# nv-nguyen/nope

Hardware: NVIDIA H100
Metric: pose-hypotheses/sec @256x256 (UNet sweep + l2 score + top-5) (higher is better)
Workload: dtype fp16

## Files before the change

### nope_b200/csrc/conv_tc.cuh

```cuda
#pragma once
#include "common.cuh"
#include <cudaTypedefs.h>

namespace nope {

constexpr int kBM = 128;
constexpr int kBK = 64;
constexpr int kMaxSeg = 64;
constexpr int kMaxAMaps = 8;
constexpr int kConvThreads = 384;
constexpr int kEpiWarps = 8;

struct ConvSeg {
  int16_t map;
  int16_t dy, dx;
  int16_t nchunks;
  int32_t wcol1;
};

struct GnFuse {
  const float* gamma;
  const float* beta;
  int G;
  int cpg;
  int gpt;
  int tpg;
  int mt;
  int ipt;
  int expected;
  int hw_shift;
  float inv_cnt;
  float eps;
  int silu;
  const __half* pb;
  int pb_stride, pb_off;
  int has_res;
  int res_div, res_base;
  int n_img;
  uint2* xpart;
  unsigned epoch;
  float2* emit;
  int emit_parts;
  __half* out_lo;
  const __half* res_lo;
  const float2* pre_stats;
  int pre_parts;
  float pre_inv_cnt;
  const float* pre_w1;
  const float* pre_wb;
  int dbg;
  unsigned long long* ts;
};

struct ConvParams {
  CUtensorMap amap[kMaxAMaps];
  int n_amaps;
  CUtensorMap bmap;
  CUtensorMap bmap2;
  CUtensorMap omap[4];
  CUtensorMap rmap;
  GnFuse gn;
  const float* bias;
  int bf16;
  int l2_prefetch;
  int n_par;
  int n_tiles_par;
  int src_w, src_hw;
  int relu;
  const __half* res_hi;
  const __half* res_lo;
  __half* out_lo;
  float* out_f32;
  int geglu;
  float2* stats;
  int stats_hw;
  int stats_noct;
  int n_total;
  int m_valid;
  int nseg;
  int ksteps;
  int m_tiles, n_tiles;
  int tiles_per_img;
  int h_cnt, b_cnt;
  ConvSeg seg[kMaxSeg];
};

template <int BN, int STAGES>
struct ConvSmem {
  static constexpr int kABytes = kBM * kBK * 2;
  static constexpr int kBBytes = BN * kBK * 2;
  static constexpr int kStageBytes = kABytes + kBBytes;
  static constexpr int kOutBytes = (BN / 64) * kBM * 128;
  static constexpr int kBarOffset = STAGES * kStageBytes + kOutBytes;
  static constexpr int kBiasOffset = kBarOffset + 256;
  static constexpr int kTotal = kBiasOffset + BN * 4 + 1024;
  static_assert(STAGES * kStageBytes >= kBM * (BN + 4) * 4, "the fp32 accumulator tile must fit in the operand ring");
  static_assert(kTotal <= 227 * 1024, "shared memory per block");
};

__device__ __forceinline__ void conv_tile_coords(const ConvParams& p, int m_tile, int& b0,
                                                 int& y0) {
  if (p.tiles_per_img > 0) {
    b0 = m_tile / p.tiles_per_img;
    y0 = (m_tile - b0 * p.tiles_per_img) * p.h_cnt;
  } else {
    b0 = m_tile * p.b_cnt;
    y0 = 0;
  }
}

__host__ __device__ constexpr int acc_ld(int BN) { return BN + 4; }

template <int NS, int STAGES, int kStageBytes, int kABytes, bool BF>
__device__ __forceinline__ void conv_mma_loop(const ConvParams& p, const uint8_t* smem, uint64_t* full_bar,
                                              uint64_t* empty_bar, int& stage, uint32_t& phase, int wg,
                                              float (&d0)[NS / 2], float (&d1)[NS / 2]) {
  const int lane = threadIdx.x & 31;
  int prev = -1;
  for (int ks = 0; ks < p.ksteps; ++ks) {
    mbar_wait(&full_bar[stage], phase);
    const uint8_t* sa = smem + stage * kStageBytes;
    const uint64_t adesc = wg_desc_k(sa);
    const uint64_t bdesc = wg_desc_k(sa + kABytes + wg * NS * 128);
    wgmma_fence();
#pragma unroll
    for (int k = 0; k < kBK / 16; ++k) {
      const uint32_t acc = (ks | k) != 0 ? 1u : 0u;
      Wgmma<NS, BF>::mma(d0, adesc + 2 * k, bdesc + 2 * k, acc);
      Wgmma<NS, BF>::mma(d1, adesc + 512 + 2 * k, bdesc + 2 * k, acc);
    }
    wgmma_commit();
    wgmma_wait<1>();
    if (prev >= 0 && lane == 0) mbar_arrive(&empty_bar[prev]);
    prev = stage;
    if (++stage == STAGES) { stage = 0; phase ^= 1; }
  }
  wgmma_wait<0>();
  if (prev >= 0 && lane == 0) mbar_arrive(&empty_bar[prev]);
}

template <int BN, int NW, int STAGES, int kStageBytes, int kABytes>
__device__ __forceinline__ void conv_mma_tile(const ConvParams& p, uint8_t* smem, uint64_t* full_bar,
                                              uint64_t* empty_bar, int& stage, uint32_t& phase, float* s_acc) {
  constexpr int NS = BN / NW;
  static_assert(NS % 32 == 0 && NS <= 128, "columns per warpgroup");
  const int wg = (threadIdx.x >> 7) - 1;
  float d0[NS / 2], d1[NS / 2];
#pragma unroll
  for (int i = 0; i < NS / 2; ++i) { d0[i] = 0.f; d1[i] = 0.f; }
  if (p.bf16) conv_mma_loop<NS, STAGES, kStageBytes, kABytes, true>(p, smem, full_bar, empty_bar, stage, phase, wg, d0, d1);
  else conv_mma_loop<NS, STAGES, kStageBytes, kABytes, false>(p, smem, full_bar, empty_bar, stage, phase, wg, d0, d1);
  asm volatile("bar.sync 2, %0;" ::"n"(NW * 128) : "memory");
  wg_store_acc<NS>(s_acc, acc_ld(BN), wg * NS, d0, d1);
  asm volatile("bar.sync 2, %0;" ::"n"(NW * 128) : "memory");
}

__device__ __forceinline__ void acc_release(uint64_t* tempty, int lane) {
  fence_proxy_async_smem();
  __syncwarp();
  if (lane == 0) mbar_arrive(tempty);
}

template <int kSeg>
__device__ __forceinline__ int butterfly8(float (&v)[8], int lane) {
  static_assert(kSeg == 16 || kSeg == 32, "segment must be 16 or 32 lanes");
  constexpr int m0 = kSeg / 2, m1 = kSeg / 4, m2 = kSeg / 8;
  {
    const bool up = (lane & m0) != 0;
#pragma unroll
    for (int i = 0; i < 4; ++i) {
      const float send = up ? v[i] : v[i + 4];
      const float keep = up ? v[i + 4] : v[i];
      v[i] = keep + __shfl_xor_sync(0xffffffffu, send, m0);
    }
  }
  {
    const bool up = (lane & m1) != 0;
#pragma unroll
    for (int i = 0; i < 2; ++i) {
      const float send = up ? v[i] : v[i + 2];
      const float keep = up ? v[i + 2] : v[i];
      v[i] = keep + __shfl_xor_sync(0xffffffffu, send, m1);
    }
  }
  {
    const bool up = (lane & m2) != 0;
    const float send = up ? v[0] : v[1];
    const float keep = up ? v[1] : v[0];
    v[0] = keep + __shfl_xor_sync(0xffffffffu, send, m2);
  }
#pragma unroll
  for (int m = m2 / 2; m > 0; m >>= 1) v[0] += __shfl_xor_sync(0xffffffffu, v[0], m);
  return ((lane & m0) ? 4 : 0) + ((lane & m1) ? 2 : 0) + ((lane & m2) ? 1 : 0);
}

template <int BN>
struct ResPrefetch {
  uint4 v[BN / 64][4];
  int next_m_tile, next_n_chan0;
  __device__ __forceinline__ void load_sub(const ConvParams& p, int cc, int m_tile, int n_chan0, int e, int lane) {
    const int q = e & 3, hh = e >> 2;
    const int grow = m_tile * kBM + q * 32 + lane;
    if (p.res_hi && m_tile >= 0 && grow < p.m_valid) {
      const size_t roff = (size_t)grow * p.n_total + n_chan0 + cc * 64 + hh * 32;
#pragma unroll
      for (int j = 0; j < 4; ++j) v[cc][j] = *reinterpret_cast<const uint4*>(p.res_hi + roff + j * 8);
    }
  }
  __device__ __forceinline__ void load(const ConvParams& p, int m_tile, int n_chan0, int e, int lane) {
#pragma unroll
    for (int cc = 0; cc < BN / 64; ++cc) load_sub(p, cc, m_tile, n_chan0, e, lane);
  }
};

template <int BN, bool EXTRAS>
__device__ __forceinline__ void conv_epilogue_tile(const ConvParams& p, uint8_t* out_stage,
                                                   const float* s_bias, const float* s_acc, int m_tile,
                                                   int n_chan0, int e, int lane,
                                                   ResPrefetch<BN>* pre = nullptr, int par = 0) {
  const int q = e & 3, hh = e >> 2;
  const int row = q * 32 + lane;
  const float* a_row = s_acc + row * acc_ld(BN) + hh * 32;
  const int grow = m_tile * kBM + row;
  const bool row_ok = grow < p.m_valid;
  size_t opix = (size_t)grow;
  if (EXTRAS && p.n_par == 4) {
    const int img = grow / p.src_hw, r = grow - img * p.src_hw;
    const int yy = r / p.src_w, xx = r - yy * p.src_w;
    opix = (size_t)img * 4 * p.src_hw + (size_t)(2 * yy + (par >> 1)) * (2 * p.src_w) + 2 * xx + (par & 1);
  }
  uint32_t v[32];
#pragma unroll
  for (int cc = 0; cc < BN / 64; ++cc) {
    acc_ld_32(a_row + cc * 64, v);
    const float* bs = s_bias + cc * 64 + hh * 32;
    uint8_t* srow = out_stage + cc * (kBM * 128) + row * 128;
    uint4 rh[4], rl[4];
    if (EXTRAS && p.res_hi && row_ok) {
      const size_t roff = (size_t)grow * p.n_total + n_chan0 + cc * 64 + hh * 32;
#pragma unroll
      for (int j = 0; j < 4; ++j) {
        rh[j] = pre ? pre->v[cc][j] : *reinterpret_cast<const uint4*>(p.res_hi + roff + j * 8);
        rl[j] = p.res_lo ? *reinterpret_cast<const uint4*>(p.res_lo + roff + j * 8) : make_uint4(0, 0, 0, 0);
      }
    }
    if (EXTRAS && pre) pre->load_sub(p, cc, pre->next_m_tile, pre->next_n_chan0, e, lane);
    float st[8];
#pragma unroll
    for (int j = 0; j < 4; ++j) {
      const float4 b0 = *reinterpret_cast<const float4*>(bs + j * 8);
      const float4 b1 = *reinterpret_cast<const float4*>(bs + j * 8 + 4);
      float f[8];
      f[0] = __uint_as_float(v[j * 8 + 0]) + b0.x;
      f[1] = __uint_as_float(v[j * 8 + 1]) + b0.y;
      f[2] = __uint_as_float(v[j * 8 + 2]) + b0.z;
      f[3] = __uint_as_float(v[j * 8 + 3]) + b0.w;
      f[4] = __uint_as_float(v[j * 8 + 4]) + b1.x;
      f[5] = __uint_as_float(v[j * 8 + 5]) + b1.y;
      f[6] = __uint_as_float(v[j * 8 + 6]) + b1.z;
      f[7] = __uint_as_float(v[j * 8 + 7]) + b1.w;
      if (EXTRAS) {
        const size_t goff = opix * p.n_total + n_chan0 + cc * 64 + hh * 32 + j * 8;
        if (p.res_hi && row_ok) {
          const __half2* h2 = reinterpret_cast<const __half2*>(&rh[j]);
          const __half2* l2 = reinterpret_cast<const __half2*>(&rl[j]);
#pragma unroll
          for (int q = 0; q < 4; ++q) {
            const float2 th = __half22float2(h2[q]), tl = __half22float2(l2[q]);
            f[2 * q] += th.x + tl.x;
            f[2 * q + 1] += th.y + tl.y;
          }
        }
        if (p.relu) {
#pragma unroll
          for (int i = 0; i < 8; ++i) f[i] = fmaxf(f[i], 0.f);
        }
        if (p.out_f32 && row_ok) {
          *reinterpret_cast<float4*>(p.out_f32 + goff) = make_float4(f[0], f[1], f[2], f[3]);
          *reinterpret_cast<float4*>(p.out_f32 + goff + 4) = make_float4(f[4], f[5], f[6], f[7]);
        }
        if (p.out_lo && row_ok) {
          float l[8];
#pragma unroll
          for (int i = 0; i < 8; ++i) l[i] = f[i] - __half2float(__float2half_rn(f[i]));
          *reinterpret_cast<uint4*>(p.out_lo + goff) =
              make_uint4(pack_half2(l[0], l[1]), pack_half2(l[2], l[3]), pack_half2(l[4], l[5]),
                         pack_half2(l[6], l[7]));
        }
      }
      float s = (f[0] + f[1]) + (f[2] + f[3]) + ((f[4] + f[5]) + (f[6] + f[7]));
      float q2 = f[0] * f[0];
#pragma unroll
      for (int i = 1; i < 8; ++i) q2 = fmaf(f[i], f[i], q2);
      st[2 * j] = s;
      st[2 * j + 1] = q2;
      const int phys = (hh * 4 + j) ^ (row & 7);
      const bool bf = p.bf16 != 0;
      *reinterpret_cast<uint4*>(srow + phys * 16) =
          make_uint4(pack2(f[0], f[1], bf), pack2(f[2], f[3], bf), pack2(f[4], f[5], bf), pack2(f[6], f[7], bf));
    }
    if (p.stats) {
      const bool small = p.stats_hw < 32;
      const int idx = small ? butterfly8<16>(st, lane) : butterfly8<32>(st, lane);
      const int seg = small ? 16 : 32;
      const int gp = m_tile * kBM + (row & ~(seg - 1));
      const bool writer = small ? ((lane & 1) == 0) : ((lane & 3) == 0);
      if (writer && gp < p.m_valid) {
        const int img = gp / p.stats_hw;
        const int parts = small ? 1 : p.stats_hw >> 5;
        const int part = small ? 0 : (gp - img * p.stats_hw) >> 5;
        float* dst = reinterpret_cast<float*>(p.stats + ((size_t)img * parts + part) * p.stats_noct +
                                              (n_chan0 + cc * 64 + hh * 32) / 8);
        dst[idx] = st[0];
      }
    }
  }
}

__device__ __forceinline__ float gelu_erf_fast(float g) {
  const float z = fabsf(g) * 0.70710678118654752f;
  const float t = __fdividef(1.f, fmaf(0.3275911f, z, 1.f));
  float poly = fmaf(t, 1.061405429f, -1.453152027f);
  poly = fmaf(poly, t, 1.421413741f);
  poly = fmaf(poly, t, -0.284496736f);
  poly = fmaf(poly, t, 0.254829592f);
  poly *= t;
  float e;
  asm("ex2.approx.ftz.f32 %0, %1;" : "=f"(e) : "f"(-z * z * 1.4426950408889634f));
  const float erf_abs = fmaf(-poly, e, 1.f);
  const float phi = 0.5f * (1.f + copysignf(erf_abs, g));
  return g * phi;
}

__device__ __forceinline__ void conv_epilogue_geglu(uint8_t* out_stage, const float* s_bias, const float* s_acc,
                                                    int e, int lane) {
  const int q = e & 3, hh = e >> 2;
  const int row = q * 32 + lane;
  const float* a_row = s_acc + row * acc_ld(128) + hh * 32;
  uint32_t vx[32], vg[32];
  acc_ld_32(a_row, vx);
  acc_ld_32(a_row + 64, vg);
  const float* bx = s_bias + hh * 32;
  const float* bg = s_bias + 64 + hh * 32;
  uint8_t* srow = out_stage + row * 128;
#pragma unroll
  for (int j = 0; j < 4; ++j) {
    float f[8];
#pragma unroll
    for (int i = 0; i < 8; ++i) {
      const float x = __uint_as_float(vx[j * 8 + i]) + bx[j * 8 + i];
      const float g = __uint_as_float(vg[j * 8 + i]) + bg[j * 8 + i];
      f[i] = x * gelu_erf_fast(g);
    }
    const int phys = (hh * 4 + j) ^ (row & 7);
    *reinterpret_cast<uint4*>(srow + phys * 16) =
        make_uint4(pack_half2(f[0], f[1]), pack_half2(f[2], f[3]), pack_half2(f[4], f[5]),
                   pack_half2(f[6], f[7]));
  }
}

template <int BN, int STAGES, bool EXTRAS>
__global__ void __launch_bounds__(kConvThreads, 1)
conv_tc_kernel(const __grid_constant__ ConvParams p) {
  using S = ConvSmem<BN, STAGES>;
  static_assert(BN % 64 == 0 && BN <= 256, "BN must be a multiple of 64");

  extern __shared__ uint8_t smem_raw[];
  uint8_t* smem = reinterpret_cast<uint8_t*>((reinterpret_cast<uintptr_t>(smem_raw) + 1023) &
                                             ~static_cast<uintptr_t>(1023));
  uint8_t* out_stage = smem + STAGES * S::kStageBytes;
  uint64_t* full_bar = reinterpret_cast<uint64_t*>(smem + S::kBarOffset);
  uint64_t* empty_bar = full_bar + STAGES;
  uint64_t* tempty_bar = empty_bar + STAGES;
  float* s_bias = reinterpret_cast<float*>(smem + S::kBiasOffset);
  float* s_acc = reinterpret_cast<float*>(smem);

  const int warp = threadIdx.x >> 5;
  const int lane = threadIdx.x & 31;
  const int num_tiles = p.m_tiles * p.n_tiles;

  if (warp == 0 && lane == 0) {
    for (int i = 0; i < p.n_amaps; ++i) prefetch_tmap(&p.amap[i]);
    prefetch_tmap(&p.bmap);
    for (int i = 0; i < p.n_par; ++i) prefetch_tmap(&p.omap[i]);
  }
  if (warp == 1 && lane == 0) {
    for (int s = 0; s < STAGES; ++s) {
      mbar_init(&full_bar[s], 1);
      mbar_init(&empty_bar[s], kEpiWarps);
    }
    mbar_init(tempty_bar, kEpiWarps);
    fence_mbar_init();
  }
  __syncthreads();

  if (warp == 0) {
    int stage = 0;
    uint32_t phase = 0;
    int iter = 0;
    for (int tile = blockIdx.x; tile < num_tiles; tile += gridDim.x, ++iter) {
      const int m_tile = tile / p.n_tiles;
      const int n_tile = tile - m_tile * p.n_tiles;
      const int par = n_tile / p.n_tiles_par;
      const int py = par >> 1, px = par & 1;
      int b0, y0;
      conv_tile_coords(p, m_tile, b0, y0);
      if (iter > 0) mbar_wait(tempty_bar, (iter - 1) & 1);
      int kcol = 0;
      for (int s = 0; s < p.nseg; ++s) {
        const ConvSeg sg = p.seg[s];
        const CUtensorMap* am = &p.amap[sg.map];
        if (sg.wcol1) kcol = sg.wcol1 - 1;
        for (int ch = 0; ch < sg.nchunks; ++ch) {
          mbar_wait(&empty_bar[stage], phase ^ 1);
          if (elect_one()) {
            uint8_t* sa = smem + stage * S::kStageBytes;
            mbar_expect_tx(&full_bar[stage], S::kStageBytes);
            tma_load_4d(sa, am, &full_bar[stage], ch * kBK, sg.dx + px, y0 + sg.dy + py, b0);
            tma_load_2d(sa + S::kABytes, &p.bmap, &full_bar[stage], kcol, n_tile * BN);
          }
          kcol += kBK;
          if (++stage == STAGES) { stage = 0; phase ^= 1; }
        }
      }
    }
  } else if (warp >= 4) {
    const int e = warp - 4;
    const int etid = threadIdx.x - 128;
    int stage = 0;
    uint32_t phase = 0;
    for (int tile = blockIdx.x; tile < num_tiles; tile += gridDim.x) {
      const int m_tile = tile / p.n_tiles;
      const int n_tile = tile - m_tile * p.n_tiles;
      const int par = n_tile / p.n_tiles_par;
      const int n_chan0 = (n_tile - par * p.n_tiles_par) * BN;
      int b0, y0;
      conv_tile_coords(p, m_tile, b0, y0);
      if (etid < BN) s_bias[etid] = p.bias ? __ldg(p.bias + n_chan0 + etid) : 0.f;
      if (etid == 0) tma_store_wait_read0();
      asm volatile("bar.sync 1, 256;" ::: "memory");
      conv_mma_tile<BN, 2, STAGES, S::kStageBytes, S::kABytes>(p, smem, full_bar, empty_bar, stage, phase, s_acc);
      conv_epilogue_tile<BN, EXTRAS>(p, out_stage, s_bias, s_acc, m_tile, n_chan0, e, lane);
      acc_release(tempty_bar, lane);
      fence_proxy_async_smem();
      asm volatile("bar.sync 1, 256;" ::: "memory");
      if (etid == 0) {
#pragma unroll 1
        for (int cc = 0; cc < BN / 64; ++cc)
          tma_store_4d(&p.omap[par], out_stage + cc * (kBM * 128), n_chan0 + cc * 64, 0, y0, b0);
        tma_store_commit();
      }
    }
    if (etid == 0) tma_store_wait_all();
  }
}

inline PFN_cuTensorMapEncodeTiled_v12000 get_encode_fn() {
  static PFN_cuTensorMapEncodeTiled_v12000 fn = nullptr;
  if (!fn) {
    void* ptr = nullptr;
    cudaDriverEntryPointQueryResult qres;
    if (cudaGetDriverEntryPoint("cuTensorMapEncodeTiled", &ptr, cudaEnableDefault, &qres) ==
            cudaSuccess &&
        qres == cudaDriverEntryPointSuccess)
      fn = reinterpret_cast<PFN_cuTensorMapEncodeTiled_v12000>(ptr);
  }
  return fn;
}

inline int make_tmap_f16(CUtensorMap* out, const void* base, int rank, const uint64_t* dims,
                         const uint64_t* strides_bytes, const uint32_t* box) {
  auto fn = get_encode_fn();
  if (!fn) return fail("cuTensorMapEncodeTiled driver entry point not available");
  cuuint64_t gdim[5], gstr[5];
  cuuint32_t bx[5], es[5];
  for (int i = 0; i < rank; ++i) { gdim[i] = dims[i]; bx[i] = box[i]; es[i] = 1; }
  for (int i = 0; i < rank - 1; ++i) gstr[i] = strides_bytes[i];
  CUresult r = fn(out, CU_TENSOR_MAP_DATA_TYPE_FLOAT16, rank, const_cast<void*>(base), gdim, gstr,
                  bx, es, CU_TENSOR_MAP_INTERLEAVE_NONE, CU_TENSOR_MAP_SWIZZLE_128B,
                  CU_TENSOR_MAP_L2_PROMOTION_L2_256B, CU_TENSOR_MAP_FLOAT_OOB_FILL_NONE);
  if (r != CUDA_SUCCESS) {
    char buf[256];
    snprintf(buf, sizeof buf,
             "cuTensorMapEncodeTiled failed (%d): rank %d dims [%llu %llu %llu %llu] box [%u %u %u %u]",
             (int)r, rank, (unsigned long long)dims[0], (unsigned long long)(rank > 1 ? dims[1] : 0),
             (unsigned long long)(rank > 2 ? dims[2] : 0), (unsigned long long)(rank > 3 ? dims[3] : 0),
             box[0], rank > 1 ? box[1] : 0, rank > 2 ? box[2] : 0, rank > 3 ? box[3] : 0);
    return fail(buf);
  }
  return 0;
}

struct TileGeom {
  int W, H, w_cnt, h_cnt, b_cnt, tiles_per_img;
};
inline int make_geom(int H, int W, TileGeom* g) {
  g->W = W; g->H = H; g->w_cnt = W;
  if (W > kBM || kBM % W != 0) return fail("conv geometry: W must divide 128");
  const int hw = H * W;
  if (hw >= kBM) {
    if (hw % kBM != 0) return fail("conv geometry: H*W must be a multiple of 128");
    g->h_cnt = kBM / W; g->b_cnt = 1; g->tiles_per_img = hw / kBM;
  } else {
    if (kBM % hw != 0) return fail("conv geometry: H*W must divide 128");
    g->h_cnt = H; g->b_cnt = kBM / hw; g->tiles_per_img = 0;
  }
  return 0;
}
inline int geom_m_tiles(const TileGeom& g, int n_img) {
  return g.tiles_per_img > 0 ? n_img * g.tiles_per_img : (n_img + g.b_cnt - 1) / g.b_cnt;
}

inline int make_act_map(CUtensorMap* m, const void* base, int cap_img, int C, const TileGeom& g) {
  uint64_t dims[4] = {(uint64_t)C, (uint64_t)g.W, (uint64_t)g.H, (uint64_t)cap_img};
  uint64_t str[3] = {(uint64_t)C * 2, (uint64_t)g.W * C * 2, (uint64_t)g.H * g.W * C * 2};
  uint32_t box[4] = {64, (uint32_t)g.w_cnt, (uint32_t)g.h_cnt, (uint32_t)g.b_cnt};
  return make_tmap_f16(m, base, 4, dims, str, box);
}
inline int make_unshuffle_map(CUtensorMap* m, const void* base, int cap_img, int C,
                              const TileGeom& g, int p1, int p2) {
  const int W2 = g.W * 2, H2 = g.H * 2;
  const uint8_t* b = static_cast<const uint8_t*>(base) + ((size_t)p1 * W2 + p2) * C * 2;
  uint64_t dims[4] = {(uint64_t)C, (uint64_t)g.W, (uint64_t)g.H, (uint64_t)cap_img};
  uint64_t str[3] = {(uint64_t)2 * C * 2, (uint64_t)2 * W2 * C * 2, (uint64_t)H2 * W2 * C * 2};
  uint32_t box[4] = {64, (uint32_t)g.w_cnt, (uint32_t)g.h_cnt, (uint32_t)g.b_cnt};
  return make_tmap_f16(m, b, 4, dims, str, box);
}
inline int make_weight_map(CUtensorMap* m, const void* base, int n_total, int k_total, int bn) {
  uint64_t dims[2] = {(uint64_t)k_total, (uint64_t)n_total};
  uint64_t str[1] = {(uint64_t)k_total * 2};
  uint32_t box[2] = {64, (uint32_t)bn};
  return make_tmap_f16(m, base, 2, dims, str, box);
}

inline int pick_bn(int n_total) {
  if (n_total % 192 == 0) return 192;
  if (n_total % 128 == 0) return 128;
  if (n_total % 64 == 0) return 64;
  return 0;
}

inline bool conv_needs_extras(const ConvParams& p) {
// ... 37 lines not shown
```

### nope_b200/csrc/conv_tc2.cuh

```cuda
#pragma once
#include "conv_tc.cuh"

namespace nope {

__device__ __forceinline__ uint32_t cluster_ctarank() {
  uint32_t r;
  asm volatile("mov.u32 %0, %%cluster_ctarank;" : "=r"(r));
  return r;
}
__device__ __forceinline__ uint32_t cluster_id_x() {
  uint32_t r;
  asm volatile("mov.u32 %0, %%clusterid.x;" : "=r"(r));
  return r;
}
__device__ __forceinline__ uint32_t num_clusters_x() {
  uint32_t r;
  asm volatile("mov.u32 %0, %%nclusterid.x;" : "=r"(r));
  return r;
}
__device__ __forceinline__ void cluster_sync_all() {
  asm volatile("barrier.cluster.arrive.release.aligned;" ::: "memory");
  asm volatile("barrier.cluster.wait.acquire.aligned;" ::: "memory");
}
__device__ __forceinline__ void tma_prefetch_4d(const CUtensorMap* m, int c0, int c1, int c2, int c3) {
  asm volatile("cp.async.bulk.prefetch.tensor.4d.L2.global.tile [%0, {%1, %2, %3, %4}];"
               ::"l"(reinterpret_cast<uint64_t>(m)), "r"(c0), "r"(c1), "r"(c2), "r"(c3)
               : "memory");
}
template <int BN>
struct Gn2Smem {
  static constexpr int kOct = BN / 8;
  static constexpr int kPart = 0;
  static constexpr int kMr = kPart + 8 * kOct * 8;
  static constexpr int kTab = kMr + 2 * 64 * 8;
  static constexpr int kOg = kTab + 2 * 2 * BN * 4;
  static constexpr int kEm = kOg + kOct * 4;
  static constexpr int kX = kEm + 2 * 32 * 8;
  static constexpr int kBytes = kX + 256 * 4;
};

template <int BN, int STAGES, int EPI = 0>
struct Conv2Smem {
  static constexpr int kABytes = kBM * kBK * 2;
  static constexpr int kBBytes = BN * kBK * 2;
  static constexpr int kStageBytes = kABytes + kBBytes;
  static constexpr int kOutBytes = (BN / 64) * kBM * 128;
  static constexpr int kOutBufs = (BN <= 128 || (EPI == 4 && STAGES <= 4)) ? 2 : 1;
  static constexpr int kBarOffset = STAGES * kStageBytes + kOutBufs * kOutBytes;
  static constexpr int kBiasOffset = kBarOffset + 256;
  static constexpr int kGnOffset = kBiasOffset + BN * 4;
  static constexpr int kGnBytes = EPI == 3 ? (2 * BN * 4 + 8 * BN * 2 + 8 * (BN / 8) * 8 + 64 * 8 + (BN / 8) * 4 + 32 * 8 + 256 * 4)
                                            : (EPI == 4 ? Gn2Smem<BN>::kBytes : 0);
  static constexpr int kTotal = kGnOffset + kGnBytes + 1024;
  static_assert(STAGES * kStageBytes >= kBM * (BN + 4) * 4, "the fp32 accumulator tile must fit in the operand ring");
  static_assert(kTotal <= 227 * 1024, "shared memory per block");
};

__device__ __forceinline__ unsigned long long global_ns() {
  unsigned long long t;
  asm volatile("mov.u64 %0, %%globaltimer;" : "=l"(t));
  return t;
}
__device__ __forceinline__ uint2 ld_volatile_u2(const uint2* p) {
  uint2 r;
  asm volatile("ld.volatile.global.v2.u32 {%0, %1}, [%2];" : "=r"(r.x), "=r"(r.y) : "l"(p) : "memory");
  return r;
}
__device__ __forceinline__ void st_volatile_u2(uint2* p, uint2 v) {
  asm volatile("st.volatile.global.v2.u32 [%0], {%1, %2};" ::"l"(p), "r"(v.x), "r"(v.y) : "memory");
}

__device__ __forceinline__ float4 lds_f4(uint32_t addr) {
  float4 r;
  asm("ld.shared.v4.f32 {%0, %1, %2, %3}, [%4];" : "=f"(r.x), "=f"(r.y), "=f"(r.z), "=f"(r.w) : "r"(addr));
  return r;
}
__device__ __forceinline__ uint4 lds_u4(uint32_t addr) {
  uint4 r;
  asm("ld.shared.v4.u32 {%0, %1, %2, %3}, [%4];" : "=r"(r.x), "=r"(r.y), "=r"(r.z), "=r"(r.w) : "r"(addr));
  return r;
}
__device__ __forceinline__ float2 lds_f2(uint32_t addr) {
  float2 r;
  asm("ld.shared.v2.f32 {%0, %1}, [%2];" : "=f"(r.x), "=f"(r.y) : "r"(addr));
  return r;
}
__device__ __forceinline__ uint32_t order_token(uint32_t v) {
  uint32_t r;
  asm volatile("mov.u32 %0, %1;" : "=r"(r) : "r"(v) : "memory");
  return r;
}

__device__ __forceinline__ float silu_ftz(float x) {
  float e, r;
  asm("ex2.approx.ftz.f32 %0, %1;" : "=f"(e) : "f"(x * -1.4426950408889634f));
  asm("rcp.approx.ftz.f32 %0, %1;" : "=f"(r) : "f"(1.0f + e));
  return x * r;
}

__host__ __device__ constexpr int gn_epi_warps(int BN) { return 4 * (BN / 64); }
__host__ __device__ constexpr int gn_threads(int BN) { return 128 + 32 * gn_epi_warps(BN); }

template <int BN, int STAGES>
__device__ __forceinline__ void conv_gn_epilogue_loop(const ConvParams& p, uint8_t* smem, uint64_t* full_bar,
                                                      uint64_t* empty_bar, uint64_t* tempty_bar, uint64_t* res_bar,
                                                      int tile0, int tile_step, int num_tiles, uint32_t rank) {
  using S = Conv2Smem<BN, STAGES, 3>;
  constexpr int kOct = BN / 8;
  constexpr int kNS = BN / 64;
  constexpr int kEpiThreads = 32 * gn_epi_warps(BN);
  uint8_t* out_stage = smem + STAGES * S::kStageBytes;
  float* s_bias = reinterpret_cast<float*>(smem + S::kBiasOffset);
  float* s_gamma = reinterpret_cast<float*>(smem + S::kGnOffset);
  float* s_beta = s_gamma + BN;
  __half* s_pb = reinterpret_cast<__half*>(s_beta + BN);
  float* s_part = reinterpret_cast<float*>(s_pb + 8 * BN);
  float2* s_mr = reinterpret_cast<float2*>(s_part + 8 * kOct * 2);
  int* s_og = reinterpret_cast<int*>(s_mr + 64);
  float2* s_em = reinterpret_cast<float2*>(s_og + kOct);
  float* s_x = reinterpret_cast<float*>(s_em + 32);

  const GnFuse& g = p.gn;
  const int warp = threadIdx.x >> 5, lane = threadIdx.x & 31;
  const int e = warp - 4, etid = threadIdx.x - 128;
  const int q = e & 3, cc = e >> 2;
  const int row = q * 32 + lane;
  const int hw = p.stats_hw;
  const bool small = hw < 32;
  const int it = hw < kBM ? (row >> g.hw_shift) : 0;
  const int npairs = g.ipt * g.gpt;
  const bool use_tab = g.G > 0 && g.ipt == 1 && g.expected > 1;
  float* s_sc = reinterpret_cast<float*>(reinterpret_cast<uint8_t*>(s_pb) + 512);
  float* s_sh = s_sc + BN;
  static_assert(512 + 2 * BN * 4 <= 8 * BN * 2, "scale / shift tables must fit behind the first pose-bias row");
  if (etid < kOct) s_og[etid] = (g.G > 0 && g.cpg < BN) ? (etid * 8) / g.cpg : 0;
#define NOPE_EPI_BAR() asm volatile("bar.sync 1, %0;" ::"n"(kEpiThreads) : "memory")

  int obuf = 0;
  uint32_t res_phase = 0;
  int iter = 0;
  int kstage = 0;
  uint32_t kphase = 0;
  float* s_acc = reinterpret_cast<float*>(smem);
  auto stage_residual = [&](int t, int buf) {
    if (t >= num_tiles) return;
    const int mp = t / p.n_tiles;
    const int nt = t - mp * p.n_tiles;
    const int mt2 = 2 * mp + (int)rank;
    if constexpr (S::kOutBufs == 2) tma_store_wait_read1();
    else tma_store_wait_read0();
    if (g.has_res && mt2 < p.m_tiles) {
      int bb, yy;
      conv_tile_coords(p, mt2, bb, yy);
      const int rb = g.res_div > 0 ? (g.res_base + bb) / g.res_div : bb;
      uint8_t* dst = out_stage + buf * S::kOutBytes;
      mbar_expect_tx(res_bar, S::kOutBytes);
#pragma unroll 1
      for (int c2 = 0; c2 < kNS; ++c2)
        tma_load_4d(dst + c2 * (kBM * 128), &p.rmap, res_bar, nt * BN + c2 * 64, 0, yy, rb);
    }
  };
  const bool res_late = (g.dbg & 8) != 0;
  if (etid == 0 && !res_late) stage_residual(tile0, 0);
  uint4 pb_next = make_uint4(0, 0, 0, 0);
  auto fetch_pb = [&](int t) {
    if (!g.pb || t >= num_tiles || etid >= g.ipt * kOct) return;
    const int mp = t / p.n_tiles;
    const int nt = t - mp * p.n_tiles;
    const int mt2 = 2 * mp + (int)rank;
    const int i0 = p.tiles_per_img > 0 ? mt2 / g.mt : mt2 * g.ipt;
    const int ii = etid / kOct, o8 = etid - ii * kOct;
    pb_next = make_uint4(0, 0, 0, 0);
    if (i0 + ii < g.n_img)
      pb_next = *reinterpret_cast<const uint4*>(g.pb + (size_t)(i0 + ii) * g.pb_stride + g.pb_off + nt * BN + o8 * 8);
  };
  static_assert(8 * kOct <= kEpiThreads, "one thread per (image, octet) of the pose-bias rows");
  fetch_pb(tile0);
#define NOPE_TS(k) do { if (g.ts && etid == 0 && iter < 64) g.ts[((size_t)blockIdx.x * 64 + iter) * 16 + (k)] = global_ns(); } while (0)
  for (int tile = tile0; tile < num_tiles; tile += tile_step, ++iter) {
    NOPE_TS(0);
    const int m_pair = tile / p.n_tiles;
    const int n_tile = tile - m_pair * p.n_tiles;
    const int m_tile = 2 * m_pair + (int)rank;
    const int n_chan0 = n_tile * BN;
    const bool live = m_tile < p.m_tiles;
    int b0, y0;
    conv_tile_coords(p, m_tile, b0, y0);
    const int img0 = p.tiles_per_img > 0 ? m_tile / g.mt : m_tile * g.ipt;
    uint8_t* ost = out_stage + obuf * S::kOutBytes;
    if (etid < BN && (tile == tile0 || p.n_tiles > 1)) {
      s_bias[etid] = p.bias ? __ldg(p.bias + n_chan0 + etid) : 0.f;
      if (g.G > 0) {
        s_gamma[etid] = __ldg(g.gamma + n_chan0 + etid);
        s_beta[etid] = __ldg(g.beta + n_chan0 + etid);
      } else if (g.pre_stats) {
        s_gamma[etid] = __ldg(g.pre_w1 + n_chan0 + etid);
        s_beta[etid] = __ldg(g.pre_wb + n_chan0 + etid);
      }
    }
    if (g.dbg & 16) fetch_pb(tile);
    if (g.pb && etid < g.ipt * kOct)
      *reinterpret_cast<uint4*>(s_pb + (etid / kOct) * BN + (etid % kOct) * 8) = pb_next;
    NOPE_EPI_BAR();
    NOPE_TS(1);
    if (!(g.dbg & 16)) fetch_pb(tile + tile_step);
    conv_mma_tile<BN, BN / 64, STAGES, S::kStageBytes, S::kABytes>(p, smem, full_bar, empty_bar, kstage, kphase, s_acc);
    NOPE_TS(2);

    uint32_t a[64];
    {
      const float* a_row = s_acc + row * acc_ld(BN) + cc * 64;
      acc_ld_32(a_row, *reinterpret_cast<uint32_t(*)[32]>(&a[0]));
      acc_ld_32(a_row + 32, *reinterpret_cast<uint32_t(*)[32]>(&a[32]));
      acc_release(tempty_bar, lane);
    }
    if (res_late && etid == 0 && (!live || g.G == 0 || g.expected == 1)) stage_residual(tile, obuf);
    if (live) {
#pragma unroll
      for (int hh = 0; hh < 2; ++hh) {
        const float* bs = s_bias + cc * 64 + hh * 32;
        float st[8];
#pragma unroll
        for (int j = 0; j < 4; ++j) {
          const float4 c0 = *reinterpret_cast<const float4*>(bs + j * 8);
          const float4 c1 = *reinterpret_cast<const float4*>(bs + j * 8 + 4);
          const float bb[8] = {c0.x, c0.y, c0.z, c0.w, c1.x, c1.y, c1.z, c1.w};
          float f[8];
#pragma unroll
          for (int i = 0; i < 8; ++i) {
            f[i] = __uint_as_float(a[hh * 32 + j * 8 + i]) + bb[i];
            a[hh * 32 + j * 8 + i] = __float_as_uint(f[i]);
          }
          float sm = (f[0] + f[1]) + (f[2] + f[3]) + ((f[4] + f[5]) + (f[6] + f[7]));
          float q2 = f[0] * f[0];
#pragma unroll
          for (int i = 1; i < 8; ++i) q2 = fmaf(f[i], f[i], q2);
          st[2 * j] = sm;
          st[2 * j + 1] = q2;
        }
        if (g.G > 0) {
          const int idx = small ? butterfly8<16>(st, lane) : butterfly8<32>(st, lane);
          const bool writer = small ? ((lane & 1) == 0) : ((lane & 3) == 0);
          const int segi = small ? (q * 2 + (lane >> 4)) : q;
          if (writer) s_part[(segi * kOct + cc * 8 + hh * 4) * 2 + idx] = st[0];
        }
      }
      if (g.G > 0) {
        NOPE_EPI_BAR();
        NOPE_TS(3);
        float Sx = 0.f, Qx = 0.f;
        if (etid < npairs) {
          const int ii = etid / g.gpt, gl = etid - ii * g.gpt;
          const int spi = hw >= kBM ? 4 : (small ? 1 : (hw >> 5));
          const int s0 = hw >= kBM ? 0 : ii * spi;
          const int opg = (g.cpg < BN ? g.cpg : BN) >> 3;
          const int o0 = gl * opg;
          for (int sgm = s0; sgm < s0 + spi; ++sgm)
            for (int o = o0; o < o0 + opg; ++o) {
              Sx += s_part[(sgm * kOct + o) * 2];
              Qx += s_part[(sgm * kOct + o) * 2 + 1];
            }
        }
        if (g.expected > 1) {
          const int sg = (m_tile / g.mt) * (p.n_tiles / g.tpg) + n_tile / g.tpg;
          const int slot = (m_tile % g.mt) * g.tpg + (n_tile % g.tpg);
          uint2* xp = g.xpart + (size_t)sg * g.expected * npairs * 2;
          if (etid < npairs) {
            st_volatile_u2(xp + ((size_t)slot * npairs + etid) * 2, make_uint2(__float_as_uint(Sx), g.epoch));
            st_volatile_u2(xp + ((size_t)slot * npairs + etid) * 2 + 1, make_uint2(__float_as_uint(Qx), g.epoch));
          }
          if (res_late && etid == 0) stage_residual(tile, obuf);
          if (etid < g.expected * npairs * 2) {
            uint2 u = ld_volatile_u2(xp + etid);
            if (u.y != g.epoch && !(g.dbg & 1)) {
              const long long t0 = clock64();
              do {
                u = ld_volatile_u2(xp + etid);
                if (clock64() - t0 > 4000000000LL) __trap();
              } while (u.y != g.epoch);
            }
            s_x[etid] = __uint_as_float(u.x);
          }
          NOPE_EPI_BAR();
          NOPE_TS(4);
          if (use_tab) {
            if (etid < BN) {
              const int gl = s_og[etid >> 3];
              float s1 = 0.f, s2 = 0.f;
              for (int sl = 0; sl < g.expected; ++sl) {
                s1 += s_x[(sl * npairs + gl) * 2];
                s2 += s_x[(sl * npairs + gl) * 2 + 1];
              }
              const float mean = s1 * g.inv_cnt;
              const float var = fmaxf(s2 * g.inv_cnt - mean * mean, 0.f);
              const float sc = rsqrtf(var + g.eps) * s_gamma[etid];
              s_sc[etid] = sc;
              s_sh[etid] = s_beta[etid] - mean * sc;
            }
          } else if (etid < npairs) {
            Sx = 0.f; Qx = 0.f;
            for (int sl = 0; sl < g.expected; ++sl) {
              Sx += s_x[(sl * npairs + etid) * 2];
              Qx += s_x[(sl * npairs + etid) * 2 + 1];
            }
          }
        }
        if (!use_tab && etid < npairs) {
          const float mean = Sx * g.inv_cnt;
          const float var = fmaxf(Qx * g.inv_cnt - mean * mean, 0.f);
          s_mr[etid] = make_float2(mean, rsqrtf(var + g.eps));
        }
        NOPE_EPI_BAR();
      }

      if (g.pre_stats) {
        if (g.ipt == 1) {
          if (etid < BN) {
            float s1 = 0.f, s2 = 0.f;
            for (int k = 0; k < g.pre_parts; ++k) {
              const float2 t = g.pre_stats[(size_t)img0 * g.pre_parts + k];
              s1 += t.x;
              s2 += t.y;
            }
            const float mean = s1 * g.pre_inv_cnt;
            const float rstd = rsqrtf(fmaxf(s2 * g.pre_inv_cnt - mean * mean, 0.f) + g.eps);
            s_sc[etid] = rstd;
            s_sh[etid] = s_beta[etid] - rstd * mean * s_gamma[etid];
          }
        } else if (etid < g.ipt) {
          float s1 = 0.f, s2 = 0.f;
          if (img0 + etid < g.n_img)
            for (int k = 0; k < g.pre_parts; ++k) {
              const float2 t = g.pre_stats[(size_t)(img0 + etid) * g.pre_parts + k];
              s1 += t.x;
              s2 += t.y;
            }
          const float mean = s1 * g.pre_inv_cnt;
          s_mr[etid] = make_float2(mean, rsqrtf(fmaxf(s2 * g.pre_inv_cnt - mean * mean, 0.f) + g.eps));
        }
        NOPE_EPI_BAR();
      }

      NOPE_TS(5);
      if (g.has_res) mbar_wait(res_bar, res_phase);
      float e1 = 0.f, e2 = 0.f;
      const uint32_t tok = order_token(smem_u32(smem));
      const uint32_t a_gamma = tok + (uint32_t)(reinterpret_cast<uint8_t*>(s_gamma) - smem) + cc * 256;
      const uint32_t a_beta = tok + (uint32_t)(reinterpret_cast<uint8_t*>(s_beta) - smem) + cc * 256;
      const uint32_t a_pb = tok + (uint32_t)(reinterpret_cast<uint8_t*>(s_pb) - smem) + (it * BN + cc * 64) * 2;
      const uint32_t a_mr = tok + (uint32_t)(reinterpret_cast<uint8_t*>(s_mr) - smem) + it * g.gpt * 8;
      const uint32_t a_sc = tok + (uint32_t)(reinterpret_cast<uint8_t*>(s_sc) - smem) + cc * 256;
      const uint32_t a_sh = tok + (uint32_t)(reinterpret_cast<uint8_t*>(s_sh) - smem) + cc * 256;
      const int grow = m_tile * kBM + row;
      const bool row_ok = grow < p.m_valid;
      const long long rpix = g.res_div > 0
          ? (long long)((g.res_base + b0) / g.res_div) * hw + (m_tile % g.mt) * kBM + row
          : (long long)grow;
      uint8_t* srow = ost + cc * (kBM * 128) + row * 128;
      const bool do_norm = g.G > 0 && !(g.dbg & 4);
// ... 85 lines not shown
      for (int j = 0; j < 8; ++j) {
        uint4 w;
        w.x = pack2(f[j * 8 + 0], f[j * 8 + 1], bf);
        w.y = pack2(f[j * 8 + 2], f[j * 8 + 3], bf);
        w.z = pack2(f[j * 8 + 4], f[j * 8 + 5], bf);
        w.w = pack2(f[j * 8 + 6], f[j * 8 + 7], bf);
        *reinterpret_cast<uint4*>(srow + ((j ^ (row & 7)) << 4)) = w;
        if (want_lo || want_emit) {
          const uint32_t* hw2 = reinterpret_cast<const uint32_t*>(&w);
          uint4 wl;
          uint32_t* pl = reinterpret_cast<uint32_t*>(&wl);
#pragma unroll
          for (int k2 = 0; k2 < 4; ++k2) {
            const float2 t = unpack2(hw2[k2], bf);
            pl[k2] = pack_half2(f[j * 8 + 2 * k2] - t.x, f[j * 8 + 2 * k2 + 1] - t.y);
            e1 += t.x + t.y;
            e2 = fmaf(t.x, t.x, e2);
            e2 = fmaf(t.y, t.y, e2);
          }
          if (want_lo)
            *reinterpret_cast<uint4*>(g.out_lo + (size_t)grow * p.n_total + n_chan0 + cc * 64 + j * 8) = wl;
        }
      }
      if (g.has_res) res_phase ^= 1;
      if (g.emit) {
#pragma unroll
        for (int off = 8; off > 0; off >>= 1) {
          e1 += __shfl_xor_sync(0xffffffffu, e1, off);
          e2 += __shfl_xor_sync(0xffffffffu, e2, off);
        }
        if ((lane & 15) == 0) s_em[cc * 8 + (row >> 4)] = make_float2(e1, e2);
        NOPE_EPI_BAR();
        if (etid < g.ipt && img0 + etid < g.n_img) {
          const int r16 = hw >= kBM ? 8 : (hw >> 4);
          float s1 = 0.f, s2 = 0.f;
          for (int h2 = 0; h2 < kNS; ++h2)
            for (int r = etid * r16; r < (etid + 1) * r16; ++r) {
              s1 += s_em[h2 * 8 + r].x;
              s2 += s_em[h2 * 8 + r].y;
            }
          g.emit[(size_t)(img0 + etid) * g.emit_parts + (m_tile % g.mt) * p.n_tiles + n_tile] = make_float2(s1, s2);
        }
      }
      fence_proxy_async_smem();
      NOPE_EPI_BAR();
      NOPE_TS(6);
      if (etid == 0) {
#pragma unroll 1
        for (int c2 = 0; c2 < kNS; ++c2)
          tma_store_4d(&p.omap[0], ost + c2 * (kBM * 128), n_chan0 + c2 * 64, 0, y0, b0);
        tma_store_commit();
      }
    }
    if (etid == 0 && !res_late) stage_residual(tile + tile_step, obuf ^ (S::kOutBufs - 1));
    obuf ^= S::kOutBufs - 1;
  }
  if (etid == 0) tma_store_wait_all();
#undef NOPE_TS
#undef NOPE_EPI_BAR
}


struct Gn2Bars {
  uint64_t* full;
  uint64_t* empty;
  uint64_t* tempty;
  uint64_t* res[2];
  uint64_t* part;
  uint64_t* stats;
  uint64_t* tabfree;
  uint64_t* out;
};

template <int NORM, bool SILU, bool PB, bool RES, bool EMIT>
__device__ __forceinline__ void gn2_pass2_octets(float* f, uint32_t a_sc, uint32_t a_sh, uint32_t a_mr, const int* og,
                                                 int it_gpt, const float4* gm4, const float4* bt4, const uint4* pb4,
                                                 bool img_ok, uint8_t* srow, uint32_t a_srow, int row, bool bf,
                                                 float& e1, float& e2) {
  float2 mr3 = make_float2(0.f, 0.f);
  if (NORM == 3) mr3 = lds_f2(a_mr);
#pragma unroll
  for (int j = 0; j < 8; ++j) {
    float* ff = f + j * 8;
    const int sw = (j ^ (row & 7)) << 4;
    uint4 rv = make_uint4(0u, 0u, 0u, 0u), pv = make_uint4(0u, 0u, 0u, 0u);
    if (RES) rv = lds_u4(a_srow + sw);
    if (PB && img_ok) pv = __ldg(pb4 + j);
    if (NORM == 1) {
      const float4 s0 = lds_f4(a_sc + j * 32), s1 = lds_f4(a_sc + j * 32 + 16);
      const float4 h0 = lds_f4(a_sh + j * 32), h1 = lds_f4(a_sh + j * 32 + 16);
      ff[0] = fmaf(ff[0], s0.x, h0.x); ff[1] = fmaf(ff[1], s0.y, h0.y);
      ff[2] = fmaf(ff[2], s0.z, h0.z); ff[3] = fmaf(ff[3], s0.w, h0.w);
      ff[4] = fmaf(ff[4], s1.x, h1.x); ff[5] = fmaf(ff[5], s1.y, h1.y);
      ff[6] = fmaf(ff[6], s1.z, h1.z); ff[7] = fmaf(ff[7], s1.w, h1.w);
    } else if (NORM == 2) {
      const float2 mr = lds_f2(a_mr + (it_gpt + og[j]) * 8);
      const float4 g0 = __ldg(gm4 + 2 * j), g1 = __ldg(gm4 + 2 * j + 1);
      const float4 t0 = __ldg(bt4 + 2 * j), t1 = __ldg(bt4 + 2 * j + 1);
      ff[0] = fmaf(ff[0] - mr.x, mr.y * g0.x, t0.x); ff[1] = fmaf(ff[1] - mr.x, mr.y * g0.y, t0.y);
      ff[2] = fmaf(ff[2] - mr.x, mr.y * g0.z, t0.z); ff[3] = fmaf(ff[3] - mr.x, mr.y * g0.w, t0.w);
      ff[4] = fmaf(ff[4] - mr.x, mr.y * g1.x, t1.x); ff[5] = fmaf(ff[5] - mr.x, mr.y * g1.y, t1.y);
      ff[6] = fmaf(ff[6] - mr.x, mr.y * g1.z, t1.z); ff[7] = fmaf(ff[7] - mr.x, mr.y * g1.w, t1.w);
    } else if (NORM == 3) {
      const float nm = -mr3.x * mr3.y;
      const float4 g0 = __ldg(gm4 + 2 * j), g1 = __ldg(gm4 + 2 * j + 1);
      const float4 t0 = __ldg(bt4 + 2 * j), t1 = __ldg(bt4 + 2 * j + 1);
      ff[0] = fmaf(ff[0], mr3.y, fmaf(nm, g0.x, t0.x)); ff[1] = fmaf(ff[1], mr3.y, fmaf(nm, g0.y, t0.y));
      ff[2] = fmaf(ff[2], mr3.y, fmaf(nm, g0.z, t0.z)); ff[3] = fmaf(ff[3], mr3.y, fmaf(nm, g0.w, t0.w));
      ff[4] = fmaf(ff[4], mr3.y, fmaf(nm, g1.x, t1.x)); ff[5] = fmaf(ff[5], mr3.y, fmaf(nm, g1.y, t1.y));
      ff[6] = fmaf(ff[6], mr3.y, fmaf(nm, g1.z, t1.z)); ff[7] = fmaf(ff[7], mr3.y, fmaf(nm, g1.w, t1.w));
    }
    if (SILU) {
#pragma unroll
      for (int i = 0; i < 8; ++i) ff[i] = silu_ftz(ff[i]);
    }
    if (PB) {
      const uint32_t* hp = reinterpret_cast<const uint32_t*>(&pv);
#pragma unroll
      for (int k2 = 0; k2 < 4; ++k2) {
        const float2 t = unpack2(hp[k2], bf);
        ff[2 * k2] += t.x;
        ff[2 * k2 + 1] += t.y;
      }
    }
    if (RES) {
      const uint32_t* hr = reinterpret_cast<const uint32_t*>(&rv);
#pragma unroll
      for (int k2 = 0; k2 < 4; ++k2) {
        const float2 t = unpack2(hr[k2], bf);
        ff[2 * k2] += t.x;
        ff[2 * k2 + 1] += t.y;
      }
    }
    uint4 w;
    w.x = pack2(ff[0], ff[1], bf);
    w.y = pack2(ff[2], ff[3], bf);
    w.z = pack2(ff[4], ff[5], bf);
    w.w = pack2(ff[6], ff[7], bf);
    *reinterpret_cast<uint4*>(srow + sw) = w;
    if (EMIT) {
      const uint32_t* hw2 = reinterpret_cast<const uint32_t*>(&w);
#pragma unroll
      for (int k2 = 0; k2 < 4; ++k2) {
        const float2 t = unpack2(hw2[k2], bf);
        e1 += t.x + t.y;
        e2 = fmaf(t.x, t.x, e2);
        e2 = fmaf(t.y, t.y, e2);
      }
    }
  }
}


template <int BN, int STAGES>
__device__ __forceinline__ void conv_gn2_math_warps(const ConvParams& p, uint8_t* smem, uint8_t* gsm,
                                                    const Gn2Bars& B, int tile0, int tile_step, int num_tiles,
                                                    uint32_t rank) {
  using S = Conv2Smem<BN, STAGES, 4>;
  using G2 = Gn2Smem<BN>;
  constexpr int kOct = BN / 8;
  constexpr int kNB = S::kOutBufs;
  uint8_t* ost0 = smem + STAGES * S::kStageBytes;
  float* s_part = reinterpret_cast<float*>(gsm + G2::kPart);
  const int* s_og = reinterpret_cast<const int*>(gsm + G2::kOg);
  float2* s_em0 = reinterpret_cast<float2*>(gsm + G2::kEm);

  const GnFuse& g = p.gn;
  const int warp = threadIdx.x >> 5, lane = threadIdx.x & 31;
  const int e = warp - 4;
  const int q = e & 3, cc = e >> 2;
  const int row = q * 32 + lane;
  const int hw = p.stats_hw;
  const bool small = hw < 32;
  const int it = hw < kBM ? (row >> g.hw_shift) : 0;
  const bool use_tab = g.G > 0 && g.ipt == 1 && g.expected > 1;
  const bool pre = g.pre_stats != nullptr;
  const bool wait_stats = g.G > 0 || pre;
  const bool bf = p.bf16 != 0;
  const uint32_t gsm_off = (uint32_t)(gsm - smem);
  int variant = -1;
  if (!(g.out_lo || g.res_lo || (g.dbg & 6))) {
    if (g.G > 0 && g.silu) {
      const int nm2 = use_tab ? 0 : 1;
      if (g.pb && !g.has_res && !g.emit) variant = nm2;
      else if (!g.pb && g.has_res) variant = 2 + 2 * nm2 + (g.emit ? 1 : 0);
    } else if (pre && g.G == 0 && !g.silu && !g.pb && !g.has_res && !g.emit) {
      variant = g.ipt > 1 ? 7 : 6;
    }
  }
  if (g.dbg & 32) variant = -1;

  int kstage = 0;
  uint32_t kphase = 0;
  float* s_acc = reinterpret_cast<float*>(smem);
  int iter = 0;
#define NOPE_TS(k) do { if (g.ts && e == 0 && lane == 0 && iter < 64) g.ts[((size_t)blockIdx.x * 64 + iter) * 16 + (k)] = global_ns(); } while (0)
  for (int tile = tile0; tile < num_tiles; tile += tile_step, ++iter) {
    NOPE_TS(0);
    const int b = iter & 1;
    const int ob = kNB == 2 ? (iter & 1) : 0;
    uint8_t* ost = ost0 + ob * S::kOutBytes;
    float2* s_em = s_em0 + ob * 32;
    const int m_pair = tile / p.n_tiles;
    const int n_tile = tile - m_pair * p.n_tiles;
    const int m_tile = 2 * m_pair + (int)rank;
    const int n_chan0 = n_tile * BN;
    const bool live = m_tile < p.m_tiles;
    int b0, y0;
    conv_tile_coords(p, m_tile, b0, y0);
    const int img0 = p.tiles_per_img > 0 ? m_tile / g.mt : m_tile * g.ipt;
    const bool img_ok = img0 + it < g.n_img;
    const __half* pb_row = g.pb + (size_t)(img_ok ? img0 + it : 0) * g.pb_stride + g.pb_off + n_chan0 + cc * 64;
    if (g.pb && live) asm volatile("prefetch.global.L1 [%0];" ::"l"(pb_row));

    conv_mma_tile<BN, BN / 64, STAGES, S::kStageBytes, S::kABytes>(p, smem, B.full, B.empty, kstage, kphase, s_acc);
    NOPE_TS(1);
    uint32_t a[64];
    {
      const float* a_row = s_acc + row * acc_ld(BN) + cc * 64;
      acc_ld_32(a_row, *reinterpret_cast<uint32_t(*)[32]>(&a[0]));
      acc_ld_32(a_row + 32, *reinterpret_cast<uint32_t(*)[32]>(&a[32]));
      acc_release(B.tempty, lane);
    }
    if (!live) continue;

    float* f = reinterpret_cast<float*>(a);
    if (p.bias) {
      const float4* b4 = reinterpret_cast<const float4*>(p.bias + n_chan0 + cc * 64);
#pragma unroll
      for (int j = 0; j < 16; ++j) {
        const float4 c = __ldg(b4 + j);
        f[4 * j + 0] += c.x;
        f[4 * j + 1] += c.y;
        f[4 * j + 2] += c.z;
        f[4 * j + 3] += c.w;
      }
    }
    if (g.G > 0) {
#pragma unroll
      for (int hh = 0; hh < 2; ++hh) {
        float st[8];
#pragma unroll
        for (int j = 0; j < 4; ++j) {
          const float* ff = f + hh * 32 + j * 8;
          const float sm = (ff[0] + ff[1]) + (ff[2] + ff[3]) + ((ff[4] + ff[5]) + (ff[6] + ff[7]));
          float q2 = ff[0] * ff[0];
#pragma unroll
          for (int i = 1; i < 8; ++i) q2 = fmaf(ff[i], ff[i], q2);
          st[2 * j] = sm;
          st[2 * j + 1] = q2;
        }
        const int idx = small ? butterfly8<16>(st, lane) : butterfly8<32>(st, lane);
        const bool writer = small ? ((lane & 1) == 0) : ((lane & 3) == 0);
        const int segi = small ? (q * 2 + (lane >> 4)) : q;
        if (writer) s_part[(segi * kOct + cc * 8 + hh * 4) * 2 + idx] = st[0];
      }
      __syncwarp();
      if (lane == 0) mbar_arrive(B.part);
    }
    NOPE_TS(2);
    if (wait_stats) mbar_wait(&B.stats[b], (iter >> 1) & 1);
    NOPE_TS(3);
    mbar_wait(B.res[ob], (iter / kNB) & 1);
    NOPE_TS(4);

    float e1 = 0.f, e2 = 0.f;
    const uint32_t tok = order_token(smem_u32(smem));
    const uint32_t a_mr = tok + gsm_off + G2::kMr + b * 64 * 8;
    const uint32_t a_sc = tok + gsm_off + G2::kTab + b * 2 * BN * 4 + cc * 256;
    const uint32_t a_sh = a_sc + BN * 4;
    const int grow = m_tile * kBM + row;
    const bool row_ok = grow < p.m_valid;
    const long long rpix = g.res_div > 0
        ? (long long)((g.res_base + b0) / g.res_div) * hw + (m_tile % g.mt) * kBM + row
        : (long long)grow;
    uint8_t* srow = ost + cc * (kBM * 128) + row * 128;
    const bool do_norm = g.G > 0 && !(g.dbg & 4);
    const bool do_silu = g.silu && !(g.dbg & 2);
    const bool want_emit = g.emit != nullptr;
    if (variant >= 0) {
      const uint32_t a_srow = tok + (uint32_t)(srow - smem);
      const float4* gm4 = reinterpret_cast<const float4*>((pre ? g.pre_w1 : g.gamma) + n_chan0 + cc * 64);
      const float4* bt4 = reinterpret_cast<const float4*>((pre ? g.pre_wb : g.beta) + n_chan0 + cc * 64);
      const uint4* pb4 = reinterpret_cast<const uint4*>(pb_row);
      const int* og = s_og + cc * 8;
      const int it_gpt = it * g.gpt;
      switch (variant) {
        case 0: gn2_pass2_octets<1, true, true, false, false>(f, a_sc, a_sh, a_mr, og, it_gpt, gm4, bt4, pb4, img_ok, srow, a_srow, row, bf, e1, e2); break;
        case 1: gn2_pass2_octets<2, true, true, false, false>(f, a_sc, a_sh, a_mr, og, it_gpt, gm4, bt4, pb4, img_ok, srow, a_srow, row, bf, e1, e2); break;
        case 2: gn2_pass2_octets<1, true, false, true, false>(f, a_sc, a_sh, a_mr, og, it_gpt, gm4, bt4, pb4, img_ok, srow, a_srow, row, bf, e1, e2); break;
        case 3: gn2_pass2_octets<1, true, false, true, true>(f, a_sc, a_sh, a_mr, og, it_gpt, gm4, bt4, pb4, img_ok, srow, a_srow, row, bf, e1, e2); break;
        case 4: gn2_pass2_octets<2, true, false, true, false>(f, a_sc, a_sh, a_mr, og, it_gpt, gm4, bt4, pb4, img_ok, srow, a_srow, row, bf, e1, e2); break;
        case 5: gn2_pass2_octets<2, true, false, true, true>(f, a_sc, a_sh, a_mr, og, it_gpt, gm4, bt4, pb4, img_ok, srow, a_srow, row, bf, e1, e2); break;
        case 6: gn2_pass2_octets<1, false, false, false, false>(f, a_sc, a_sh, a_mr, og, it_gpt, gm4, bt4, pb4, img_ok, srow, a_srow, row, bf, e1, e2); break;
        default: gn2_pass2_octets<3, false, false, false, false>(f, a_sc, a_sh, a_mr + it * 8, og, it_gpt, gm4, bt4, pb4, img_ok, srow, a_srow, row, bf, e1, e2); break;
      }
    } else {
    if (pre && g.ipt > 1) {
      const float2 mr = lds_f2(a_mr + it * 8);
      const float nm = -mr.x * mr.y;
      const float4* w14 = reinterpret_cast<const float4*>(g.pre_w1 + n_chan0 + cc * 64);
      const float4* wb4 = reinterpret_cast<const float4*>(g.pre_wb + n_chan0 + cc * 64);
#pragma unroll
      for (int j = 0; j < 16; ++j) {
        const float4 w1 = __ldg(w14 + j), wb = __ldg(wb4 + j);
        f[4 * j + 0] = fmaf(f[4 * j + 0], mr.y, fmaf(nm, w1.x, wb.x));
        f[4 * j + 1] = fmaf(f[4 * j + 1], mr.y, fmaf(nm, w1.y, wb.y));
        f[4 * j + 2] = fmaf(f[4 * j + 2], mr.y, fmaf(nm, w1.z, wb.z));
        f[4 * j + 3] = fmaf(f[4 * j + 3], mr.y, fmaf(nm, w1.w, wb.w));
      }
    } else if ((do_norm && use_tab) || pre) {
#pragma unroll
      for (int j = 0; j < 16; ++j) {
        const float4 sc = lds_f4(a_sc + j * 16), sh = lds_f4(a_sh + j * 16);
        f[4 * j + 0] = fmaf(f[4 * j + 0], sc.x, sh.x);
        f[4 * j + 1] = fmaf(f[4 * j + 1], sc.y, sh.y);
        f[4 * j + 2] = fmaf(f[4 * j + 2], sc.z, sh.z);
        f[4 * j + 3] = fmaf(f[4 * j + 3], sc.w, sh.w);
      }
    } else if (do_norm) {
      const float4* gm4 = reinterpret_cast<const float4*>(g.gamma + n_chan0 + cc * 64);
      const float4* bt4 = reinterpret_cast<const float4*>(g.beta + n_chan0 + cc * 64);
#pragma unroll
      for (int j = 0; j < 8; ++j) {
        const float2 mr = lds_f2(a_mr + (it * g.gpt + s_og[cc * 8 + j]) * 8);
#pragma unroll
        for (int h2 = 0; h2 < 2; ++h2) {
          const float4 gm = __ldg(gm4 + j * 2 + h2), bt = __ldg(bt4 + j * 2 + h2);
          float* ff = f + j * 8 + h2 * 4;
          ff[0] = fmaf(ff[0] - mr.x, mr.y * gm.x, bt.x);
          ff[1] = fmaf(ff[1] - mr.x, mr.y * gm.y, bt.y);
          ff[2] = fmaf(ff[2] - mr.x, mr.y * gm.z, bt.z);
          ff[3] = fmaf(ff[3] - mr.x, mr.y * gm.w, bt.w);
        }
      }
    }
    if (do_silu) {
#pragma unroll
      for (int i = 0; i < 64; ++i) f[i] = silu_ftz(f[i]);
    }
    if (g.pb && img_ok) {
      const uint4* pb4 = reinterpret_cast<const uint4*>(pb_row);
#pragma unroll
      for (int j = 0; j < 8; ++j) {
        const uint4 pv = __ldg(pb4 + j);
        const uint32_t* hp = reinterpret_cast<const uint32_t*>(&pv);
#pragma unroll
        for (int k2 = 0; k2 < 4; ++k2) {
          const float2 t = unpack2(hp[k2], bf);
          f[j * 8 + 2 * k2] += t.x;
          f[j * 8 + 2 * k2 + 1] += t.y;
        }
      }
    }
    if (g.has_res) {
#pragma unroll
      for (int j = 0; j < 8; ++j) {
        const uint4 rv = *reinterpret_cast<const uint4*>(srow + ((j ^ (row & 7)) << 4));
        const uint32_t* hr = reinterpret_cast<const uint32_t*>(&rv);
#pragma unroll
        for (int k2 = 0; k2 < 4; ++k2) {
          const float2 t = unpack2(hr[k2], bf);
          f[j * 8 + 2 * k2] += t.x;
          f[j * 8 + 2 * k2 + 1] += t.y;
        }
      }
      if (g.res_lo && row_ok) {
#pragma unroll
// ... 239 lines not shown
            const float var = fmaxf(s2 * g.inv_cnt - mean * mean, 0.f);
            const float sc = rsqrtf(var + g.eps) * __ldg(g.gamma + n_chan0 + c);
            t_sc[c] = sc;
            t_sh[c] = __ldg(g.beta + n_chan0 + c) - mean * sc;
          }
        } else {
#pragma unroll
          for (int k = 0; k < 2; ++k) {
            const int pr = lane + 32 * k;
            if (pr < npairs) {
              float S1 = 0.f, S2 = 0.f;
              for (int sl = 0; sl < g.expected; ++sl) {
                S1 += s_x[(sl * npairs + pr) * 2];
                S2 += s_x[(sl * npairs + pr) * 2 + 1];
              }
              const float mean = S1 * g.inv_cnt;
              const float var = fmaxf(S2 * g.inv_cnt - mean * mean, 0.f);
              mr[pr] = make_float2(mean, rsqrtf(var + g.eps));
            }
          }
        }
      } else {
#pragma unroll
        for (int k = 0; k < 2; ++k) {
          const int pr = lane + 32 * k;
          if (pr < npairs) {
            const float mean = Sx[k] * g.inv_cnt;
            const float var = fmaxf(Qx[k] * g.inv_cnt - mean * mean, 0.f);
            mr[pr] = make_float2(mean, rsqrtf(var + g.eps));
          }
        }
      }
    }
    if (pre) {
      if (g.ipt == 1) {
        float s1 = 0.f, s2 = 0.f;
        for (int k0 = 0; k0 < g.pre_parts; k0 += 32) {
          float2 t = make_float2(0.f, 0.f);
          if (k0 + lane < g.pre_parts) t = g.pre_stats[(size_t)img0 * g.pre_parts + k0 + lane];
          const int n = g.pre_parts - k0 < 32 ? g.pre_parts - k0 : 32;
          for (int k = 0; k < n; ++k) {
            s1 += __shfl_sync(0xffffffffu, t.x, k);
            s2 += __shfl_sync(0xffffffffu, t.y, k);
          }
        }
        const float mean = s1 * g.pre_inv_cnt;
        const float rstd = rsqrtf(fmaxf(s2 * g.pre_inv_cnt - mean * mean, 0.f) + g.eps);
#pragma unroll
        for (int c = lane; c < BN; c += 32) {
          t_sc[c] = rstd;
          t_sh[c] = __ldg(g.pre_wb + n_chan0 + c) - rstd * mean * __ldg(g.pre_w1 + n_chan0 + c);
        }
      } else if (lane < g.ipt) {
        float2 t[8];
#pragma unroll
        for (int k = 0; k < 8; ++k) {
          t[k] = make_float2(0.f, 0.f);
          if (k < g.pre_parts && img0 + lane < g.n_img) t[k] = g.pre_stats[(size_t)(img0 + lane) * g.pre_parts + k];
        }
        float s1 = 0.f, s2 = 0.f;
#pragma unroll
        for (int k = 0; k < 8; ++k)
          if (k < g.pre_parts) {
            s1 += t[k].x;
            s2 += t[k].y;
          }
        const float mean = s1 * g.pre_inv_cnt;
        mr[lane] = make_float2(mean, rsqrtf(fmaxf(s2 * g.pre_inv_cnt - mean * mean, 0.f) + g.eps));
      }
    }
    __syncwarp();
    if (lane == 0) mbar_arrive(&B.stats[b]);
    NOPE_TS2(12);
  }
#undef NOPE_TS2
}

template <int BN, int STAGES>
__device__ __forceinline__ void conv_gn2_store_warp(const ConvParams& p, uint8_t* smem, uint8_t* gsm, const Gn2Bars& B,
                                                    int tile0, int tile_step, int num_tiles, uint32_t rank) {
  using S = Conv2Smem<BN, STAGES, 4>;
  using G2 = Gn2Smem<BN>;
  constexpr int kNS = BN / 64;
  constexpr int kNB = S::kOutBufs;
  uint8_t* ost0 = smem + STAGES * S::kStageBytes;
  const float2* s_em0 = reinterpret_cast<const float2*>(gsm + G2::kEm);
  const GnFuse& g = p.gn;
  const int lane = threadIdx.x & 31;
  const int hw = p.stats_hw;
  auto stage = [&](int t, int ob) {
    if (t >= num_tiles) return;
    const int mp = t / p.n_tiles;
    const int nt = t - mp * p.n_tiles;
    const int mt2 = 2 * mp + (int)rank;
    if (g.has_res && mt2 < p.m_tiles) {
      int bb, yy;
      conv_tile_coords(p, mt2, bb, yy);
      const int rb = g.res_div > 0 ? (g.res_base + bb) / g.res_div : bb;
      uint8_t* dst = ost0 + ob * S::kOutBytes;
      mbar_expect_tx(B.res[ob], S::kOutBytes);
#pragma unroll 1
      for (int c2 = 0; c2 < kNS; ++c2)
        tma_load_4d(dst + c2 * (kBM * 128), &p.rmap, B.res[ob], nt * BN + c2 * 64, 0, yy, rb);
    } else {
      mbar_arrive(B.res[ob]);
    }
  };
  if (lane == 0) {
    stage(tile0, 0);
    if (kNB == 2) stage(tile0 + tile_step, 1);
  }
  int iter = 0;
  for (int tile = tile0; tile < num_tiles; tile += tile_step, ++iter) {
    const int ob = kNB == 2 ? (iter & 1) : 0;
    const int m_pair = tile / p.n_tiles;
    const int n_tile = tile - m_pair * p.n_tiles;
    const int m_tile = 2 * m_pair + (int)rank;
    if (m_tile >= p.m_tiles) break;
    int b0, y0;
    conv_tile_coords(p, m_tile, b0, y0);
    const int img0 = p.tiles_per_img > 0 ? m_tile / g.mt : m_tile * g.ipt;
    mbar_wait(&B.out[ob], (iter / kNB) & 1);
    if (g.ts && lane == 0 && iter < 64) g.ts[((size_t)blockIdx.x * 64 + iter) * 16 + 13] = global_ns();
    if (g.emit && lane < g.ipt && img0 + lane < g.n_img) {
      const float2* s_em = s_em0 + ob * 32;
      const int r16 = hw >= kBM ? 8 : (hw >> 4);
      float s1 = 0.f, s2 = 0.f;
      for (int h2 = 0; h2 < kNS; ++h2)
        for (int r = lane * r16; r < (lane + 1) * r16; ++r) {
          s1 += s_em[h2 * 8 + r].x;
          s2 += s_em[h2 * 8 + r].y;
        }
      g.emit[(size_t)(img0 + lane) * g.emit_parts + (m_tile % g.mt) * p.n_tiles + n_tile] = make_float2(s1, s2);
    }
    __syncwarp();
    if (lane == 0) {
      uint8_t* ost = ost0 + ob * S::kOutBytes;
#pragma unroll 1
      for (int c2 = 0; c2 < kNS; ++c2)
        tma_store_4d(&p.omap[0], ost + c2 * (kBM * 128), n_tile * BN + c2 * 64, 0, y0, b0);
      tma_store_commit();
      const int nt = tile + kNB * tile_step;
      if (nt < num_tiles) {
        tma_store_wait_read0();
        if (g.ts && iter < 64) g.ts[((size_t)blockIdx.x * 64 + iter) * 16 + 14] = global_ns();
        stage(nt, ob);
      }
    }
    __syncwarp();
  }
  if (lane == 0) tma_store_wait_all();
}

template <int BN, int STAGES, int EPI>
__global__ void __cluster_dims__(2, 1, 1) __launch_bounds__(EPI >= 3 ? gn_threads(BN) : kConvThreads, 1)
conv_tc2_kernel(const __grid_constant__ ConvParams p) {
  using S = Conv2Smem<BN, STAGES, EPI>;
  static_assert(BN % 64 == 0 && BN <= 256, "BN must be a multiple of 64");
  constexpr int kMathWarps = EPI >= 3 ? gn_epi_warps(BN) : kEpiWarps;

  extern __shared__ uint8_t smem_raw[];
  uint8_t* smem = reinterpret_cast<uint8_t*>((reinterpret_cast<uintptr_t>(smem_raw) + 1023) &
                                             ~static_cast<uintptr_t>(1023));
  uint8_t* out_stage = smem + STAGES * S::kStageBytes;
  uint64_t* full_bar = reinterpret_cast<uint64_t*>(smem + S::kBarOffset);
  uint64_t* empty_bar = full_bar + STAGES;
  uint64_t* tempty_bar = empty_bar + STAGES;
  uint64_t* res_bar = tempty_bar + 1;
  uint64_t* gn2_bar = res_bar + 1;
  static_assert((2 * STAGES + 2 + 8) * 8 <= 256, "barrier block overflow");
  float* s_bias = reinterpret_cast<float*>(smem + S::kBiasOffset);
  float* s_acc = reinterpret_cast<float*>(smem);

  const int warp = threadIdx.x >> 5;
  const int lane = threadIdx.x & 31;
  const uint32_t rank = cluster_ctarank();
  const int m_pairs = (p.m_tiles + 1) >> 1;
  const int num_tiles = m_pairs * p.n_tiles;
  const int tile0 = cluster_id_x(), tile_step = num_clusters_x();

  if (warp == 0 && lane == 0) {
    for (int i = 0; i < p.n_amaps; ++i) prefetch_tmap(&p.amap[i]);
    prefetch_tmap(&p.bmap2);
    for (int i = 0; i < p.n_par; ++i) prefetch_tmap(&p.omap[i]);
  }
  if (warp == 1 && lane == 0) {
    for (int s = 0; s < STAGES; ++s) {
      mbar_init(&full_bar[s], 1);
      mbar_init(&empty_bar[s], kMathWarps);
    }
    mbar_init(tempty_bar, kMathWarps);
    mbar_init(res_bar, 1);
    if constexpr (EPI == 4) {
      mbar_init(&gn2_bar[0], gn_epi_warps(BN));
      mbar_init(&gn2_bar[1], 1);
      mbar_init(&gn2_bar[2], 1);
      mbar_init(&gn2_bar[3], gn_epi_warps(BN));
      mbar_init(&gn2_bar[4], gn_epi_warps(BN));
      mbar_init(&gn2_bar[5], gn_epi_warps(BN));
      mbar_init(&gn2_bar[6], gn_epi_warps(BN));
      mbar_init(&gn2_bar[7], 1);
    }
    fence_mbar_init();
  }
  __syncthreads();
  pdl_sync();

  if (warp == 0) {
    int stage = 0;
    uint32_t phase = 0;
    int iter = 0;
    for (int tile = tile0; tile < num_tiles; tile += tile_step, ++iter) {
      const int m_pair = tile / p.n_tiles;
      const int n_tile = tile - m_pair * p.n_tiles;
      const int m_tile = 2 * m_pair + (int)rank;
      const int par = n_tile / p.n_tiles_par;
      const int py = par >> 1, px = par & 1;
      int b0, y0;
      conv_tile_coords(p, m_tile, b0, y0);
      if (iter > 0) mbar_wait(tempty_bar, (iter - 1) & 1);
      if (p.l2_prefetch && tile + tile_step < num_tiles) {
        const int nt = tile + tile_step;
        const int nmp = nt / p.n_tiles;
        if (nmp != m_pair) {
          const int nmt = 2 * nmp + (int)rank;
          int nb0, ny0;
          conv_tile_coords(p, nmt, nb0, ny0);
          if (nmt < p.m_tiles && elect_one()) {
            for (int s = 0; s < p.nseg; ++s) {
              const ConvSeg sg = p.seg[s];
              if (sg.dy != 0 || sg.dx != 0) continue;
              for (int ch = 0; ch < sg.nchunks; ++ch) tma_prefetch_4d(&p.amap[sg.map], ch * kBK, 0, ny0, nb0);
            }
          }
          __syncwarp();
        }
      }
      int kcol = 0;
      for (int s = 0; s < p.nseg; ++s) {
        const ConvSeg sg = p.seg[s];
        const CUtensorMap* am = &p.amap[sg.map];
        if (sg.wcol1) kcol = sg.wcol1 - 1;
        for (int ch = 0; ch < sg.nchunks; ++ch) {
          mbar_wait(&empty_bar[stage], phase ^ 1);
          if (elect_one()) {
            uint8_t* sa = smem + stage * S::kStageBytes;
            mbar_expect_tx(&full_bar[stage], S::kStageBytes);
            tma_load_4d(sa, am, &full_bar[stage], ch * kBK, sg.dx + px, y0 + sg.dy + py, b0);
            tma_load_2d(sa + S::kABytes, &p.bmap2, &full_bar[stage], kcol, n_tile * BN);
          }
          kcol += kBK;
          if (++stage == STAGES) { stage = 0; phase ^= 1; }
        }
      }
    }
  } else if (EPI == 4 && warp >= 2) {
    if constexpr (EPI == 4) {
      Gn2Bars B;
      B.full = full_bar; B.empty = empty_bar; B.tempty = tempty_bar; B.res[0] = res_bar; B.res[1] = &gn2_bar[7];
      B.part = &gn2_bar[0]; B.stats = &gn2_bar[1]; B.tabfree = &gn2_bar[3]; B.out = &gn2_bar[5];
      uint8_t* gsm = smem + S::kGnOffset;
      if (warp == 2) conv_gn2_store_warp<BN, STAGES>(p, smem, gsm, B, tile0, tile_step, num_tiles, rank);
      else if (warp == 3) conv_gn2_stats_warp<BN, STAGES>(p, gsm, B, tile0, tile_step, num_tiles, rank);
      else conv_gn2_math_warps<BN, STAGES>(p, smem, gsm, B, tile0, tile_step, num_tiles, rank);
    }
  } else if (warp >= 4 && EPI == 3) {
    if constexpr (EPI == 3)
      conv_gn_epilogue_loop<BN, STAGES>(p, smem, full_bar, empty_bar, tempty_bar, res_bar, tile0, tile_step,
                                        num_tiles, rank);
  } else if (warp >= 4) {
    const int e = warp - 4;
    const int etid = threadIdx.x - 128;
    int kstage = 0;
    uint32_t kphase = 0;
    int obuf = 0;
    constexpr bool kPrefetchRes = EPI == 1 && BN <= 128;
    ResPrefetch<kPrefetchRes ? BN : 64> pre;
    if constexpr (kPrefetchRes) {
      if (tile0 < num_tiles) {
        const int mp0 = tile0 / p.n_tiles;
        pre.load(p, 2 * mp0 + (int)rank, (tile0 - mp0 * p.n_tiles) * BN, e, lane);
      }
    }
    for (int tile = tile0; tile < num_tiles; tile += tile_step) {
      const int m_pair = tile / p.n_tiles;
      const int n_tile = tile - m_pair * p.n_tiles;
      const int m_tile = 2 * m_pair + (int)rank;
      const int par = n_tile / p.n_tiles_par;
      const int n_chan0 = (n_tile - par * p.n_tiles_par) * BN;
      int b0, y0;
      conv_tile_coords(p, m_tile, b0, y0);
      if (etid < BN) s_bias[etid] = p.bias ? __ldg(p.bias + n_chan0 + etid) : 0.f;
      if constexpr (kPrefetchRes) {
        const int nt = tile + tile_step;
        const int nmp = nt / p.n_tiles;
        pre.next_m_tile = nt < num_tiles ? 2 * nmp + (int)rank : -1;
        pre.next_n_chan0 = (nt - nmp * p.n_tiles) * BN;
      }
      uint8_t* ost = out_stage + obuf * S::kOutBytes;
      if (etid == 0) {
        if constexpr (S::kOutBufs == 2) tma_store_wait_read1();
        else tma_store_wait_read0();
      }
      asm volatile("bar.sync 1, 256;" ::: "memory");
      conv_mma_tile<BN, 2, STAGES, S::kStageBytes, S::kABytes>(p, smem, full_bar, empty_bar, kstage, kphase, s_acc);
      if constexpr (EPI == 2)
        conv_epilogue_geglu(ost, s_bias, s_acc, e, lane);
      else if constexpr (kPrefetchRes)
        conv_epilogue_tile<BN, true>(p, ost, s_bias, s_acc, m_tile, n_chan0, e, lane, &pre);
      else if constexpr (EPI == 1)
        conv_epilogue_tile<BN, true>(p, ost, s_bias, s_acc, m_tile, n_chan0, e, lane, nullptr, par);
      else
        conv_epilogue_tile<BN, false>(p, ost, s_bias, s_acc, m_tile, n_chan0, e, lane);
      acc_release(tempty_bar, lane);
      fence_proxy_async_smem();
      asm volatile("bar.sync 1, 256;" ::: "memory");
      if (etid == 0) {
        if constexpr (EPI == 2) {
          tma_store_4d(&p.omap[0], ost, n_chan0 / 2, 0, y0, b0);
        } else {
#pragma unroll 1
          for (int cc = 0; cc < BN / 64; ++cc)
            tma_store_4d(&p.omap[par], ost + cc * (kBM * 128), n_chan0 + cc * 64, 0, y0, b0);
        }
        tma_store_commit();
      }
      obuf ^= S::kOutBufs - 1;
    }
    if (etid == 0) tma_store_wait_all();
  }
}

template <int BN, int STAGES, int EPI>
inline int launch_conv_tc2_t(const ConvParams& p, int num_sms, cudaStream_t stream) {
  using S = Conv2Smem<BN, STAGES, EPI>;
  static int max_clusters_of[kMaxDevices];
  int dev = 0;
  NOPE_CUDA(cudaGetDevice(&dev));
  NOPE_CHECK(dev >= 0 && dev < kMaxDevices, "device index out of range");
  if (max_clusters_of[dev] == 0) {
    if (const char* e = getenv("NOPE_MBAR_HINT")) {
      const uint32_t v = (uint32_t)atoi(e);
      NOPE_CUDA(cudaMemcpyToSymbol(c_mbar_suspend_ns, &v, sizeof v));
    }
    NOPE_CUDA(cudaFuncSetAttribute(conv_tc2_kernel<BN, STAGES, EPI>,
                                   cudaFuncAttributeMaxDynamicSharedMemorySize, S::kTotal));
    int mc = num_sms / 2;
    if (EPI >= 3) {
      cudaLaunchConfig_t cfg;
      memset(&cfg, 0, sizeof cfg);
      cfg.gridDim = dim3(num_sms, 1, 1);
      cfg.blockDim = dim3(EPI >= 3 ? gn_threads(BN) : kConvThreads, 1, 1);
      cfg.dynamicSmemBytes = S::kTotal;
      cudaLaunchAttribute at;
      at.id = cudaLaunchAttributeClusterDimension;
      at.val.clusterDim.x = 2; at.val.clusterDim.y = 1; at.val.clusterDim.z = 1;
      cfg.attrs = &at;
      cfg.numAttrs = 1;
      int n = 0;
      NOPE_CUDA(cudaOccupancyMaxActiveClusters(&n, conv_tc2_kernel<BN, STAGES, EPI>, &cfg));
      NOPE_CHECK(n >= 1, "conv_tc2_kernel: no resident cluster fits on this device");
      if (n < mc) mc = n;
    }
    max_clusters_of[dev] = mc;
  }
  const int pair_tiles = ((p.m_tiles + 1) / 2) * p.n_tiles;
  const int max_clusters = max_clusters_of[dev];
  const int clusters = pair_tiles < max_clusters ? pair_tiles : max_clusters;
  cudaLaunchConfig_t cfg;
  memset(&cfg, 0, sizeof cfg);
  cfg.gridDim = dim3(2 * clusters, 1, 1);
  cfg.blockDim = dim3(EPI >= 3 ? gn_threads(BN) : kConvThreads, 1, 1);
  cfg.dynamicSmemBytes = S::kTotal;
  cfg.stream = stream;
  cudaLaunchAttribute at;
  at.id = cudaLaunchAttributeProgrammaticStreamSerialization;
  at.val.programmaticStreamSerializationAllowed = 1;
  cfg.attrs = &at;
  cfg.numAttrs = (pdl_mask() & 1) ? 1 : 0;
  NOPE_CUDA(cudaLaunchKernelEx(&cfg, conv_tc2_kernel<BN, STAGES, EPI>, p));
  return 0;
}

inline int launch_conv_gn(const ConvParams& p, int bn, int num_sms, cudaStream_t stream) {
  if (p.n_par != 1 || p.geglu || conv_needs_extras(p) || p.stats)
    return fail("launch_conv_gn: the fused GroupNorm epilogue takes a plain convolution");
  static const int epi = [] {
    const char* e = getenv("NOPE_GN_EPI");
    return e && atoi(e) == 3 ? 3 : 4;
  }();
  if (epi == 3) {
    switch (bn) {
      case 192: return launch_conv_tc2_t<192, 4, 3>(p, num_sms, stream);
      case 128: return launch_conv_tc2_t<128, 4, 3>(p, num_sms, stream);
      case 64: return launch_conv_tc2_t<64, 6, 3>(p, num_sms, stream);
    }
  } else {
    switch (bn) {
      case 192: return launch_conv_tc2_t<192, 3, 4>(p, num_sms, stream);
      case 128: return launch_conv_tc2_t<128, 4, 4>(p, num_sms, stream);
      case 64: return launch_conv_tc2_t<64, 7, 4>(p, num_sms, stream);
    }
  }
  return fail("launch_conv_gn: unsupported BN");
}

inline int launch_conv_tc2(const ConvParams& p, int bn, int num_sms, cudaStream_t stream) {
  const bool ex = conv_needs_extras(p);
  if (p.geglu) {
    if (bn != 128 || ex || p.stats || p.n_par != 1) return fail("launch_conv_tc2: GEGLU epilogue needs BN = 128, no extras");
    return launch_conv_tc2_t<128, 5, 2>(p, num_sms, stream);
  }
  switch (bn) {
    case 256: return ex ? launch_conv_tc2_t<256, 3, 1>(p, num_sms, stream)
                        : launch_conv_tc2_t<256, 3, 0>(p, num_sms, stream);
    case 192: return ex ? launch_conv_tc2_t<192, 4, 1>(p, num_sms, stream)
                        : launch_conv_tc2_t<192, 4, 0>(p, num_sms, stream);
    case 128: return ex ? launch_conv_tc2_t<128, 5, 1>(p, num_sms, stream)
                        : launch_conv_tc2_t<128, 5, 0>(p, num_sms, stream);
    case 64: return ex ? launch_conv_tc2_t<64, 8, 1>(p, num_sms, stream)
                       : launch_conv_tc2_t<64, 8, 0>(p, num_sms, stream);
  }
  return fail("launch_conv_tc2: unsupported BN");
}

}
```

### nope_b200/csrc/nope_b200.cu

```cuda
#include "../../include/nope_b200.h"

#include <algorithm>
#include <cstdio>
#include <cstdlib>
#include <cstring>
#include <map>
#include <memory>
#include <string>
#include <tuple>
#include <vector>

#include "common.cuh"
#include "conv_tc.cuh"
#include "conv_tc2.cuh"
#include "kernels.cuh"
#include "linattn_tc.cuh"
#include "encoder.cuh"
#include "ldm.cuh"

using namespace nope;

namespace {

constexpr int kAbiVersion = 2;
// ... 580 lines not shown
        add_seg(mh0, t, c0 / 64, L.K + wbase);
        if (in1.hi) add_seg(map_index(0, 1, 0), t, c1 / 64, L.K + wbase + c0);
      }
      if (alo0) add_seg(ml0, t, c0 / 64, wbase);
      if (alo1) add_seg(map_index(0, 1, 1), t, c1 / 64, wbase + c0);
    }
    p.bmap = L.wmap;
    p.bmap2 = L.wmap;
    p.bf16 = bf() ? 1 : 0;
    static const int l2pf = std::getenv("NOPE_L2_PREFETCH") ? std::atoi(std::getenv("NOPE_L2_PREFETCH")) : 0;
    p.l2_prefetch = l2pf;
    if (L.mode == 3) {
      for (int t = 0; t < 4; ++t) {
        if (get_map(&m, out.hi, cap_img, L.cout, g, t)) return -1;
        p.omap[t] = *m;
      }
      p.src_w = g.W;
      p.src_hw = g.H * g.W;
    } else {
      if (get_map(&m, out.hi, cap_img, L.cout, g, -1)) return -1;
      for (int t = 0; t < 4; ++t) p.omap[t] = *m;
    }
    p.bias = L.bias;
    p.stats = stats;
    p.stats_hw = So * So;
    p.stats_noct = L.cout / 8;
    p.n_total = L.cout;
    p.m_valid = n_img * g.H * g.W;
    p.nseg = nseg;
    p.ksteps = ksteps;
    p.m_tiles = geom_m_tiles(g, n_img);
    p.n_tiles_par = L.cout / L.bn;
    p.n_tiles = p.n_tiles_par * p.n_par;
    p.tiles_per_img = g.tiles_per_img;
    p.h_cnt = g.h_cnt;
    p.b_cnt = g.b_cnt;
    NOPE_CHECK(!(stats && L.mode == 3), "fused statistics are not available on the upsample conv");
    if (gs) {
      NOPE_CHECK(conv_impl == 2 && L.mode != 3 && !stats, "fused GroupNorm epilogue: CTA-pair kernel, no upsample");
      GnFuse& f = p.gn;
      const int hw = So * So;
      f.G = gs->norm ? gs->norm->G : 0;
      if (gs->norm) {
        NOPE_CHECK(gs->norm->C == L.cout, "fused GroupNorm: channel mismatch");
        f.gamma = gs->norm->gamma;
        f.beta = gs->norm->beta;
        f.cpg = L.cout / f.G;
        NOPE_CHECK(f.cpg % 8 == 0 && (f.cpg >= L.bn ? f.cpg % L.bn == 0 : L.bn % f.cpg == 0),
                   "fused GroupNorm: groups must tile the channel tiles");
      } else {
        f.cpg = L.cout;
      }
      f.gpt = std::max(1, L.bn / f.cpg);
      f.tpg = std::max(1, f.cpg / L.bn);
      f.mt = std::max(1, g.tiles_per_img);
      f.ipt = g.tiles_per_img > 0 ? 1 : g.b_cnt;
      f.expected = f.G > 0 ? f.mt * f.tpg : 1;
      int sh = 0;
      while ((1 << sh) < hw) ++sh;
      NOPE_CHECK((1 << sh) == hw, "fused GroupNorm: H*W must be a power of two");
      f.hw_shift = sh;
      f.inv_cnt = 1.0f / ((float)hw * (float)f.cpg);
      f.eps = 1e-5f;
      f.silu = gs->silu ? 1 : 0;
      f.pb = gs->pb_offset >= 0 ? pb : nullptr;
      f.pb_stride = P;
      f.pb_off = std::max(gs->pb_offset, 0);
      f.n_img = n_img;
      if (gs->res.hi) {
        NOPE_CHECK(gs->res.C == L.cout, "fused residual: channel mismatch");
        NOPE_CHECK(gs->res_div == 0 || g.tiles_per_img > 0, "residual image mapping needs >= 128-pixel images");
        if (get_map(&m, gs->res.hi, gs->res_div > 0 ? cap_ref : cap_img, L.cout, g, -1)) return -1;
        p.rmap = *m;
        f.has_res = 1;
        f.res_lo = gs->res.lo;
      } else {
        p.rmap = p.omap[0];
      }
      f.res_div = gs->res_div;
      f.res_base = gs->res_base;
      if (gs->pre_stats) {
        NOPE_CHECK(!gs->norm && L.pre_w1 && L.pre_wb && L.mode == 1 && !L.bias, "pre-norm fold: bias-free 1x1 layer with folded weights");
        f.pre_stats = gs->pre_stats;
        f.pre_parts = gs->pre_parts;
        f.pre_inv_cnt = 1.0f / ((float)hw * (float)L.cin);
        f.pre_w1 = L.pre_w1;
        f.pre_wb = L.pre_wb;
      }
      f.out_lo = out.lo;
      static const int dbg = std::getenv("NOPE_GN_DBG") ? std::atoi(std::getenv("NOPE_GN_DBG")) : 0;
      f.dbg = dbg;
      f.emit = gs->emit;
      f.emit_parts = f.mt * p.n_tiles;
      NOPE_CHECK(f.ipt * f.gpt <= 64 && f.ipt <= 8, "fused GroupNorm: tile holds too many (image, group) pairs");
      if (f.expected > 1) {
        const size_t n_sg = (size_t)(p.m_tiles / f.mt + 1) * (p.n_tiles / f.tpg);
        NOPE_CHECK(xpart && f.expected * f.ipt * f.gpt * 2 <= 256, "fused GroupNorm: sync group too large");
        NOPE_CHECK(n_sg * f.expected * f.ipt * f.gpt * 2 <= xpart_words, "fused GroupNorm: partial-sum buffer too small");
        f.xpart = xpart;
        if (++gn_epoch == 0) ++gn_epoch;
        f.epoch = gn_epoch;
      }
    } else if (out.lo) {
      p.out_lo = out.lo;
    }
    unsigned long long* ts_dev = nullptr;
    if (gs) {
      static const int ts_k = std::getenv("NOPE_GN_TS") ? std::atoi(std::getenv("NOPE_GN_TS")) : -1;
      static int ts_count = 0;
      if (ts_k >= 0 && ts_count++ == ts_k) {
        cudaMalloc(reinterpret_cast<void**>(&ts_dev), (size_t)num_sms * 64 * 16 * sizeof(unsigned long long));
        cudaMemset(ts_dev, 0, (size_t)num_sms * 64 * 16 * sizeof(unsigned long long));
        p.gn.ts = ts_dev;
      }
    }
    auto launch = [&]() {
      if (gs) return launch_conv_gn(p, L.bn, num_sms, st);
      return conv_impl == 2 ? launch_conv_tc2(p, L.bn, num_sms, st) : launch_conv_tc(p, L.bn, num_sms, st);
    };
    if (ts_dev) {
      const int rc = launch();
      cudaDeviceSynchronize();
      std::vector<unsigned long long> h((size_t)num_sms * 64 * 16);
      cudaMemcpy(h.data(), ts_dev, h.size() * sizeof(unsigned long long), cudaMemcpyDeviceToHost);
      cudaFree(ts_dev);
      if (FILE* f = std::fopen(std::getenv("NOPE_GN_TS_FILE") ? std::getenv("NOPE_GN_TS_FILE") : "gn_ts.csv", "w")) {
        std::fprintf(f, "# So=%d n_img=%d cout=%d K=%d expected=%d m_tiles=%d n_tiles=%d\n", So, n_img, L.cout, L.K,
                     p.gn.expected, p.m_tiles, p.n_tiles);
        for (int c = 0; c < num_sms; ++c)
          for (int it = 0; it < 64; ++it) {
            const unsigned long long* r = &h[((size_t)c * 64 + it) * 16];
            if (r[0] == 0) continue;
            {
              std::fprintf(f, "%d,%d", c, it);
              for (int k = 0; k < 16; ++k) std::fprintf(f, ",%llu", r[k]);
              std::fprintf(f, "\n");
            }
          }
        std::fclose(f);
      }
      return rc;
    }
    if (!profile) return launch();
    cudaEvent_t e0, e1;
    NOPE_CUDA(cudaEventCreate(&e0));
    NOPE_CUDA(cudaEventCreate(&e1));
    NOPE_CUDA(cudaEventRecord(e0, st));
    const int rc = launch();
    NOPE_CUDA(cudaEventRecord(e1, st));
    prof_ev.push_back(e0);
    prof_ev.push_back(e1);
    prof_flops.push_back(2.0 * (double)n_img * So * So * (double)L.cout * (double)ksteps * 64.0);
    prof_alg.push_back(2.0 * (double)n_img * So * So * (double)L.cout * (double)L.K);
    return rc;
  }
  std::vector<double> prof_alg;

  static int gn_nslab(int hw, int n_img) {
    int ns = 1;
    while (ns < 8 && hw / (ns * 2) >= 32 && (long long)n_img * ns < 600) ns *= 2;
    return ns;
  }

  int gn(const NormLayer* N, const __half* x, __half* y, int S, int C, int n_img, bool silu,
         int pb_offset, const __half* res, const int* res_map, cudaStream_t st,
         const float2* stats = nullptr, int st_parts = 0, int st_noct = 0, float2* emit = nullptr) {
    const int hw = S * S;
    const int nslab = gn_nslab(hw, n_img);
    const int threads = (C / 8) * gn_rows(C);
    NOPE_CHECK(threads <= 1024 && threads % 32 == 0 && threads >= 256 && C % 8 == 0,
               "gn: unsupported channel count");
    if (N) {
      NOPE_CHECK(N->C == C, "gn: channel mismatch");
      if (!stats) {
        gn_stats_kernel<<<dim3(nslab, n_img), threads, threads * sizeof(float2), st>>>(
            x, gn_partial, hw, C, N->G, nslab);
        NOPE_CUDA(cudaGetLastError());
        ++launches;
        stats = gn_partial;
        st_parts = nslab;
        st_noct = N->G;
      }
      NOPE_CHECK(st_noct % N->G == 0, "gn: statistics granularity does not match the groups");
    }
    GnApplyArgs a;
    a.x = x; a.y = y; a.stats = N ? stats : nullptr; a.st_parts = st_parts; a.st_noct = st_noct;
    a.gamma = N ? N->gamma : nullptr; a.beta = N ? N->beta : nullptr;
    a.pb = pb_offset >= 0 ? pb : nullptr; a.pb_stride = P; a.pb_off = pb_offset >= 0 ? pb_offset : 0;
    a.res = res; a.res_of = res_map; a.emit = emit; a.emit_parts = emit_parts_of(hw);
    a.hw = hw; a.C = C; a.G = N ? N->G : 1; a.nslab = nslab;
    a.silu = silu ? 1 : 0; a.eps = 1e-5f; a.bf16 = bf() ? 1 : 0;
    NOPE_CUDA(launch_gn_apply(a, dim3(nslab, n_img), threads, st));
    ++launches;
    return 0;
  }
  static int st_parts_of(int S) { return S * S < 32 ? 1 : S * S / 32; }
  static int emit_parts_of(int hw) { return hw >= 256 ? 8 : (hw >= 32 ? hw / 32 : 1); }
  static int fused_emit_parts(int S, int C) {
    return std::max(1, S * S / kBM) * (C / pick_bn(C));
  }

  int tap(const char* name, const Act& buf, int C, int S, int n, cudaStream_t st) {
    if (tap_out == nullptr || tap_name != name || tap_hit) return 0;
    NOPE_CHECK((int64_t)n * C * S * S <= tap_cap, "debug tap: output buffer too small");
    nhwc_f16_to_nchw_f32_kernel<<<ew_grid((long long)n * C * S * S), 256, 0, st>>>(buf.hi, tap_out, n, C, S * S,
                                                                                   buf.lo, bf());
    NOPE_CUDA(cudaGetLastError());
    tap_C = C; tap_S = S; tap_hit = true;
    return 0;
  }

  int resblock(const std::string& p, const Act& in0, const Act& in1, const Act& out, int S, int n, bool pose,
               cudaStream_t st, bool emit_g1 = false, int res_div = 0, int res_base = 0, const Act* hoisted_h = nullptr) {
    const ConvLayer& b1 = convs.at(p + ".block1");
    const ConvLayer& b2 = convs.at(p + ".block2");
    const int co = b1.cout;
    const int parts = st_parts_of(S);
    auto it = convs.find(p + ".res");
    if (fused()) {
      Act h(TB.hi, co, h_lo() ? TB.lo : nullptr);
      if (hoisted_h) {
        h = *hoisted_h;
        if (!h_lo()) h.lo = nullptr;
      } else {
        GnSpec s1;
        s1.norm = &norms.at(p + ".norm1");
        s1.silu = true;
        s1.pb_offset = pose ? pb_off.at(p) : -1;
        if (conv(b1, in0, in1, h, S, n, cap, st, nullptr, &s1)) return -1;
      }
      GnSpec s2;
      s2.norm = &norms.at(p + ".norm2");
      s2.silu = true;
      if (it != convs.end()) {
        Act r(TC.hi, co, split() ? TC.lo : nullptr);
        static const bool plain_via_gn = std::getenv("NOPE_PLAIN_EPI4") && std::atoi(std::getenv("NOPE_PLAIN_EPI4"));
        GnSpec s0;
        if (conv(it->second, in0, in1, r, S, n, cap, st, nullptr, plain_via_gn ? &s0 : nullptr)) return -1;
        s2.res = r;
      } else {
        NOPE_CHECK(in1.hi == nullptr && in0.C == co, "resblock: identity residual needs Cin == Cout");
        s2.res = in0;
        s2.res_div = res_div;
        s2.res_base = res_base;
      }
      s2.emit = emit_g1 ? SB : nullptr;
      return conv(b2, h, Act(), out, S, n, cap, st, nullptr, &s2);
    }
    NOPE_CHECK(!hoisted_h && res_div == 0, "resblock: hoisting arguments belong to the fused schedule");
    if (conv(b1, in0, in1, Act(TA.hi, co), S, n, cap, st, SA)) return -1;
    if (gn(&norms.at(p + ".norm1"), TA.hi, TB.hi, S, co, n, true, pose ? pb_off.at(p) : -1, nullptr, nullptr, st,
           SA, parts, co / 8))
      return -1;
    if (conv(b2, Act(TB.hi, co), Act(), Act(TA.hi, co), S, n, cap, st, SA)) return -1;
    const __half* res = in0.hi;
    if (it != convs.end()) {
      if (conv(it->second, in0, in1, Act(TC.hi, co), S, n, cap, st)) return -1;
      res = TC.hi;
    } else {
      NOPE_CHECK(in1.hi == nullptr && in0.C == co, "resblock: identity residual needs Cin == Cout");
    }
    return gn(&norms.at(p + ".norm2"), TA.hi, out.hi, S, co, n, true, -1, res, nullptr, st, SA, parts, co / 8,
              emit_g1 ? SB : nullptr);
  }

  int linattn(const std::string& p, const Act& x, const Act& out, int C, int S, int n, cudaStream_t st) {
    const int eparts = fused() ? fused_emit_parts(S, C) : emit_parts_of(S * S);
    if (fused()) {
      GnSpec s;
      s.pre_stats = SB;
      s.pre_parts = eparts;
      if (conv(convs.at(p + ".qkvf"), x, Act(), Act(TD.hi, 3 * kHeadsHidden), S, n, cap, st, nullptr, &s)) return -1;
    } else {
      if (gn(&norms.at(p + ".prenorm"), x.hi, TB.hi, S, C, n, false, -1, nullptr, nullptr, st, SB, eparts, 1))
        return -1;
      if (conv(convs.at(p + ".qkv"), Act(TB.hi, C), Act(), Act(TD.hi, 3 * kHeadsHidden), S, n, cap, st)) return -1;
    }
    if (attn_impl == 0 && S * S >= kBM) {
      if (launch_linattn_tc(TD.hi, TC.hi, n, S * S, num_sms, st, bf())) return -1;
    } else {
      NOPE_CUDA(launch_pdl(linattn_kernel, dim3(4, n), dim3(kLinAttnThreads), 0, st, TD.hi, TC.hi, S * S, bf()));
    }
    ++launches;
    static const bool fuse_to_out = !(std::getenv("NOPE_FUSE_TO_OUT") && !std::atoi(std::getenv("NOPE_FUSE_TO_OUT")));
    if (fused() && (split() || fuse_to_out)) {
      GnSpec s;
      s.norm = &norms.at(p + ".outnorm");
      s.res = x;
      return conv(convs.at(p + ".out"), Act(TC.hi, kHeadsHidden), Act(), out, S, n, cap, st, nullptr, &s);
    }
    if (conv(convs.at(p + ".out"), Act(TC.hi, kHeadsHidden), Act(), Act(TA.hi, C), S, n, cap, st, SA)) return -1;
    return gn(&norms.at(p + ".outnorm"), TA.hi, out.hi, S, C, n, false, -1, x.hi, nullptr, st, SA, st_parts_of(S),
              C / 8);
  }

  int midattn(const Act& x, const Act& out, int C, int S, int n, cudaStream_t st) {
    NOPE_CHECK(S * S <= 32, "bottleneck attention supports at most 32 tokens");
    const int eparts = fused() ? fused_emit_parts(S, C) : emit_parts_of(S * S);
    if (fused()) {
      GnSpec s;
      s.pre_stats = SB;
      s.pre_parts = eparts;
      if (conv(convs.at("mid_attn.qkvf"), x, Act(), Act(TD.hi, 3 * kHeadsHidden), S, n, cap, st, nullptr, &s)) return -1;
    } else {
      if (gn(&norms.at("mid_attn.prenorm"), x.hi, TB.hi, S, C, n, false, -1, nullptr, nullptr, st, SB, eparts, 1))
        return -1;
      if (conv(convs.at("mid_attn.qkv"), Act(TB.hi, C), Act(), Act(TD.hi, 3 * kHeadsHidden), S, n, cap, st)) return -1;
    }
    NOPE_CUDA(launch_pdl(midattn_kernel, dim3(n), dim3(128), 0, st, TD.hi, TC.hi, S * S, bf()));
// ... 132 lines not shown

int nope_unet::iota_div(int* r, int h0, int N, int n, cudaStream_t st) {
  iota_div_kernel<<<(n + 255) / 256, 256, 0, st>>>(r, h0, N, n);
  ++launches;
  return 0;
}

namespace {
struct Scratch {
  std::vector<void*> p;
  ~Scratch() { for (void* q : p) cudaFree(q); }
  template <typename T> int get(T** out, size_t n) {
    NOPE_CUDA(cudaMalloc(reinterpret_cast<void**>(out), std::max<size_t>(n, 1) * sizeof(T)));
    p.push_back(*out);
    return 0;
  }
};
int to_nhwc(const float* x, __half** out, Scratch& s, int n, int C, int hw, cudaStream_t st,
            __half** out_lo = nullptr) {
  if (s.get(out, (size_t)n * C * hw)) return -1;
  if (out_lo && s.get(out_lo, (size_t)n * C * hw)) return -1;
  nchw_f32_to_nhwc_f16_kernel<<<ew_grid((long long)n * C * hw), 256, 0, st>>>(x, *out, n, C, hw,
                                                                              out_lo ? *out_lo : nullptr);
  NOPE_CUDA(cudaGetLastError());
  return 0;
}
int to_nchw(const __half* x, float* out, int n, int C, int hw, cudaStream_t st, const __half* x_lo = nullptr) {
  nhwc_f16_to_nchw_f32_kernel<<<ew_grid((long long)n * C * hw), 256, 0, st>>>(x, out, n, C, hw, x_lo);
  NOPE_CUDA(cudaGetLastError());
  return 0;
}
}

extern "C" {

const char* nope_last_error(void) { return last_error().c_str(); }
int nope_abi_version(void) { return kAbiVersion; }
const char* nope_build_arch(void) { return "sm_90a"; }

int nope_unet_create(nope_unet_t** out, int u_net_dim, int latent_ch, int latent_hw, int device) {
  NOPE_CHECK(out != nullptr, "null out pointer");
  NOPE_CHECK(u_net_dim > 0 && u_net_dim % 64 == 0, "u_net_dim must be a positive multiple of 64");
  NOPE_CHECK(latent_ch >= 1 && latent_ch <= kMaxLatent, "latent_ch must be in [1, 8]");
  NOPE_CHECK(latent_hw == 32, "latent_hw must be 32 (256x256 images) in this build");
  int ndev = 0;
  NOPE_CUDA(cudaGetDeviceCount(&ndev));
  NOPE_CHECK(device >= 0 && device < ndev, "no such CUDA device");
  cudaDeviceProp prop;
  NOPE_CUDA(cudaGetDeviceProperties(&prop, device));
  NOPE_CHECK(prop.major == 9 && prop.minor == 0, "nope_b200 kernels are built for sm_90a (H100) only");
  auto u = std::make_unique<nope_unet>();
  u->dim = u_net_dim;
  u->Cl = latent_ch;
  u->S0 = latent_hw;
  u->cemb = 4 * u_net_dim;
  u->device = device;
  u->num_sms = prop.multiProcessorCount;
  const int mults[4] = {1, 2, 4, 8};
  u->dims[0] = u_net_dim;
  for (int i = 0; i < 4; ++i) u->dims[i + 1] = u_net_dim * mults[i];
  u->build_schema();
  *out = u.release();
  return 0;
}

void nope_unet_destroy(nope_unet_t* u) { delete u; }

int nope_unet_load_tensor(nope_unet_t* u, const char* key, const float* data, const int64_t* shape,
                          int ndim) {
  NOPE_CHECK(u && key && data && shape, "null argument");
  NOPE_CHECK(!u->finalized, "engine already finalized");
  auto it = u->expected.find(key);
  NOPE_CHECK(it != u->expected.end(), std::string("unexpected state_dict key: ") + key);
  NOPE_CHECK((int)it->second.size() == ndim, std::string("rank mismatch for ") + key);
  size_t n = 1;
  for (int i = 0; i < ndim; ++i) {
    NOPE_CHECK(it->second[i] == shape[i], std::string("shape mismatch for ") + key);
    n *= (size_t)shape[i];
  }
  HostTensor t;
  t.shape.assign(shape, shape + ndim);
  t.data.assign(data, data + n);
  u->host[key] = std::move(t);
  return 0;
}

int nope_unet_finalize(nope_unet_t* u) {
  NOPE_CHECK(u, "null engine");
  return u->finalize();
}

int nope_unet_set_chunk(nope_unet_t* u, int hyps) {
  NOPE_CHECK(u && hyps >= 1 && hyps <= 4096, "chunk must be in [1, 4096]");
  u->chunk = hyps;
  return 0;
}
int nope_unet_set_conv_impl(nope_unet_t* u, int impl) {
  NOPE_CHECK(u && impl >= 0 && impl <= 2, "impl must be 0 (tensor cores), 1 (simt) or 2 (tensor cores, clustered)");
  NOPE_CHECK(impl != 1 || u->precision == 0, "the SIMT debug convolution only runs fp16 weights");
  u->conv_impl = impl;
  return 0;
}
int nope_unet_set_option(nope_unet_t* u, const char* name, int value) {
  NOPE_CHECK(u && name, "null argument");
  if (std::strcmp(name, "fuse_gn") == 0) {
    NOPE_CHECK(value != 0 || u->precision < 2, "split precision / bf16 need the fused GroupNorm epilogue");
    u->fuse_gn = value != 0;
    return 0;
  }
  if (std::strcmp(name, "precision") == 0) {
    NOPE_CHECK(!u->finalized, "precision must be set before nope_unet_finalize");
    NOPE_CHECK(value == 0 || u->conv_impl != 1, "the SIMT debug convolution only runs fp16 weights");
    NOPE_CHECK(value >= 0 && value <= 4, "precision must be 0 (fp16), 1 (exact weights), 2 (split), 3 (bf16) or 4 (split, fp16 inside ResnetBlocks)");
    u->precision = value;
    return 0;
  }
  if (std::strcmp(name, "conv_impl") == 0) return nope_unet_set_conv_impl(u, value);
  if (std::strcmp(name, "attn_impl") == 0) {
    NOPE_CHECK(value == 0 || value == 1, "attn_impl must be 0 (tensor cores) or 1 (CUDA cores)");
    u->attn_impl = value;
    return 0;
  }
  return fail(std::string("unknown option: ") + name);
}
int nope_unet_get_option(const nope_unet_t* u, const char* name, int* value) {
  NOPE_CHECK(u && name && value, "null argument");
  if (std::strcmp(name, "fuse_gn") == 0) { *value = u->fuse_gn ? 1 : 0; return 0; }
  if (std::strcmp(name, "precision") == 0) { *value = u->precision; return 0; }
  if (std::strcmp(name, "conv_impl") == 0) { *value = u->conv_impl; return 0; }
  if (std::strcmp(name, "attn_impl") == 0) { *value = u->attn_impl; return 0; }
  return fail(std::string("unknown option: ") + name);
}
int64_t nope_unet_last_launch_count(const nope_unet_t* u) { return u ? u->launches : 0; }

int64_t nope_unet_workspace_bytes(nope_unet_t* u, int hyps, int refs, int scores) {
  if (!u || !u->finalized || hyps < 1 || refs < 1 || scores < 0) {
    fail("nope_unet_workspace_bytes: finalized engine, hyps >= 1, refs >= 1 required");
    return -1;
  }
  return (int64_t)u->workspace_bytes(hyps, refs, scores);
}
int nope_unet_set_workspace(nope_unet_t* u, void* ptr, int64_t bytes, int hyps, int refs, int scores) {
  NOPE_CHECK(u && u->finalized, "engine not finalized");
  NOPE_CUDA(cudaSetDevice(u->device));
  return u->set_workspace(ptr, (size_t)bytes, hyps, refs, scores);
}

int nope_unet_profile(nope_unet_t* u, int enable) {
  NOPE_CHECK(u, "null engine");
  for (cudaEvent_t e : u->prof_ev) cudaEventDestroy(e);
  u->prof_ev.clear();
  u->prof_flops.clear();
  u->prof_alg.clear();
  u->profile = enable != 0;
  return 0;
}

int nope_unet_profile_read(nope_unet_t* u, double* conv_ms, double* conv_flops, double* conv_alg_flops,
                           int64_t* conv_launches, double* max_launch_tflops) {
  NOPE_CHECK(u && conv_ms && conv_flops && conv_launches, "null argument");
  NOPE_CUDA(cudaDeviceSynchronize());
  double ms = 0.0, fl = 0.0, alg = 0.0, best = 0.0;
  for (size_t i = 0; i < u->prof_flops.size(); ++i) {
    float t = 0.f;
    NOPE_CUDA(cudaEventElapsedTime(&t, u->prof_ev[2 * i], u->prof_ev[2 * i + 1]));
    ms += t;
    fl += u->prof_flops[i];
    alg += u->prof_alg[i];
    if (t > 0.f) best = std::max(best, u->prof_flops[i] / (t * 1e-3) / 1e12);
  }
  if (const char* path = std::getenv("NOPE_PROF_DUMP")) {
    if (FILE* f = std::fopen(path, "a")) {
      std::fprintf(f, "# launch,ms,executed_gflop,algorithmic_gflop\n");
      for (size_t i = 0; i < u->prof_flops.size(); ++i) {
        float t = 0.f;
        cudaEventElapsedTime(&t, u->prof_ev[2 * i], u->prof_ev[2 * i + 1]);
        std::fprintf(f, "%zu,%.4f,%.3f,%.3f\n", i, t, u->prof_flops[i] / 1e9, u->prof_alg[i] / 1e9);
      }
      std::fclose(f);
    }
  }
  *conv_ms = ms;
  *conv_flops = fl;
  if (conv_alg_flops) *conv_alg_flops = alg;
  *conv_launches = (int64_t)u->prof_flops.size();
  if (max_launch_tflops) *max_launch_tflops = best;
  return 0;
}

int nope_unet_sweep(nope_unet_t* u, const float* ref_feat, const float* poses, int B, int N,
                    const float* query_feat, float* out_emb, float* out_sim, int k, float* out_topv,
                    int64_t* out_topi, int64_t idx_base, void* stream) {
  NOPE_CHECK(u && u->finalized, "engine not finalized");
  NOPE_CHECK(ref_feat && poses && B >= 1 && N >= 1, "bad arguments");
  NOPE_CHECK(!(out_sim || k > 0) || query_feat, "scores / top-k need query_feat");
  NOPE_CHECK(k >= 0 && k <= N && k <= 64, "k must be in [0, min(N, 64)]");
  NOPE_CHECK(k == 0 || (out_topv && out_topi), "top-k outputs missing");
  cudaStream_t st = static_cast<cudaStream_t>(stream);
  NOPE_CUDA(cudaSetDevice(u->device));
  u->launches = 0;
  const int total = B * N;
  const int cap = std::min(u->chunk, total);
  if (u->ensure_workspace(cap, B, query_feat ? total : 0)) return -1;
  if (u->prepare_stream(st)) return -1;
  const int hw = u->S0 * u->S0;
  const int nslab = (hw + kFinalPix - 1) / kFinalPix;
  float* part = query_feat ? u->score_partial : nullptr;
  if (u->prestage(ref_feat, B, st)) return -1;
  for (int h0 = 0; h0 < total; h0 += cap) {
    const int n = std::min(cap, total - h0);
    if (u->forward_chunk(poses, h0, n, N, query_feat, out_emb, part, st)) return -1;
  }
  if (query_feat && (out_sim || k > 0)) {
    float* sim = out_sim ? out_sim : u->sim_buf;
    NOPE_CUDA(launch_pdl(sim_topk_kernel, dim3(B), dim3(256), 0, st, part, nslab, sim, N, k, out_topv,
                         reinterpret_cast<long long*>(out_topi), (long long)idx_base, kScoreParts, u->metric, hw));
    ++u->launches;
  }
  return 0;
}

int nope_unet_set_metric(nope_unet_t* u, int metric, float occlusion_threshold) {
  NOPE_CHECK(u, "null engine");
  NOPE_CHECK(metric == NOPE_METRIC_L2 || metric == NOPE_METRIC_COSINE || metric == NOPE_METRIC_COSINE_OCC,
             "unknown similarity metric (l2, cosine and cosine_occlusion exist)");
  u->metric = metric;
  u->occ_threshold = occlusion_threshold;
  return 0;
}

int nope_score_topk(const float* query_feat, const float* emb, int B, int N, int C, int HW, int metric,
                    float occlusion_threshold, int k, float* out_sim, float* out_topv, int64_t* out_topi,
                    int64_t idx_base, void* stream) {
  NOPE_CHECK(query_feat && emb && out_sim, "null argument");
  NOPE_CHECK(metric == NOPE_METRIC_L2 || metric == NOPE_METRIC_COSINE || metric == NOPE_METRIC_COSINE_OCC,
             "unknown similarity metric (l2, cosine and cosine_occlusion exist)");
  NOPE_CHECK(k >= 0 && k <= N && k <= 64, "k must be in [0, min(N, 64)]");
  NOPE_CHECK(k == 0 || (out_topv && out_topi), "top-k outputs missing");
  cudaStream_t st = static_cast<cudaStream_t>(stream);
  score_kernel<<<dim3(N, B), 256, 0, st>>>(query_feat, emb, out_sim, N, C, HW, metric, occlusion_threshold);
  NOPE_CUDA(cudaGetLastError());
  if (k > 0) {
    sim_topk_kernel<<<B, 256, 0, st>>>(nullptr, 0, out_sim, N, k, out_topv,
                                       reinterpret_cast<long long*>(out_topi), (long long)idx_base);
    NOPE_CUDA(cudaGetLastError());
  }
  return 0;
}

int nope_topk(float* sim, int B, int N, int k, float* out_topv, int64_t* out_topi, int64_t idx_base,
              void* stream) {
  NOPE_CHECK(sim && out_topv && out_topi, "null argument");
  NOPE_CHECK(k >= 1 && k <= N && k <= 64, "k must be in [1, min(N, 64)]");
  sim_topk_kernel<<<B, 256, 0, static_cast<cudaStream_t>(stream)>>>(
      nullptr, 0, sim, N, k, out_topv, reinterpret_cast<long long*>(out_topi), (long long)idx_base);
  NOPE_CUDA(cudaGetLastError());
  return 0;
}

int64_t nope_topk_pack_floats(int B, int k, int n_local_max, int want_sim) {
  if (B < 1 || k < 1 || n_local_max < 0) return -1;
  const int64_t kk = ((int64_t)B * k + 1) & ~(int64_t)1;
  return (kk + 2 * (int64_t)B * k + (want_sim ? (int64_t)B * n_local_max : 0) + 3) & ~(int64_t)3;
}

int nope_topk_merge(const float* gathered, int world, int64_t pack_floats, int B, int k, int N, int per,
                    int has_sim, float* out_sim, float* out_topv, int64_t* out_topi, void* stream) {
  NOPE_CHECK(gathered && out_topv && out_topi, "null argument");
  NOPE_CHECK(world >= 1 && B >= 1 && k >= 1 && k <= N && world * k <= 1024, "bad merge geometry (world * k <= 1024)");
  NOPE_CHECK(per >= 1 && (int64_t)per * world >= N, "per-rank pose count does not cover the grid");
  NOPE_CHECK(pack_floats >= nope_topk_pack_floats(B, k, has_sim ? per : 0, has_sim) - 3, "packed record too short");
  NOPE_CHECK(pack_floats % 2 == 0 && (reinterpret_cast<uintptr_t>(gathered) & 7) == 0,
             "packed records must be 8-byte aligned: use nope_topk_pack_floats for the record length");
  NOPE_CHECK(!has_sim || out_sim, "similarity output missing");
  topk_merge_kernel<<<B, 256, 0, static_cast<cudaStream_t>(stream)>>>(
      gathered, world, (long long)pack_floats, B, k, N, per, has_sim, out_sim, out_topv,
      reinterpret_cast<long long*>(out_topi));
  NOPE_CUDA(cudaGetLastError());
  return 0;
}

int nope_encoder_create(nope_encoder_t** out, int descriptor_size, int device) {
  NOPE_CHECK(out != nullptr, "null out pointer");
  NOPE_CHECK(descriptor_size >= 1 && descriptor_size <= 64, "descriptor_size must be in [1, 64]");
  int ndev = 0;
  NOPE_CUDA(cudaGetDeviceCount(&ndev));
  NOPE_CHECK(device >= 0 && device < ndev, "no such CUDA device");
  cudaDeviceProp prop;
  NOPE_CUDA(cudaGetDeviceProperties(&prop, device));
  NOPE_CHECK(prop.major == 9 && prop.minor == 0, "nope_b200 kernels are built for sm_90a (H100) only");
  auto e = std::make_unique<nope_encoder>();
  e->D = descriptor_size;
  e->device = device;
  e->num_sms = prop.multiProcessorCount;
  e->build_schema();
  *out = e.release();
  return 0;
}

void nope_encoder_destroy(nope_encoder_t* e) { delete e; }

int nope_encoder_load_tensor(nope_encoder_t* e, const char* key, const float* data, const int64_t* shape,
                             int ndim) {
  NOPE_CHECK(e && key && data && shape, "null argument");
  NOPE_CHECK(!e->finalized, "encoder already finalized");
  auto it = e->expected.find(key);
  NOPE_CHECK(it != e->expected.end(), std::string("unexpected encoder state_dict key: ") + key);
  NOPE_CHECK((int)it->second.size() == ndim, std::string("rank mismatch for ") + key);
  size_t n = 1;
  for (int i = 0; i < ndim; ++i) {
    NOPE_CHECK(it->second[i] == shape[i], std::string("shape mismatch for ") + key);
    n *= (size_t)shape[i];
  }
  auto& slot = e->host[key];
  slot.first.assign(shape, shape + ndim);
  slot.second.assign(data, data + n);
  return 0;
}

int nope_encoder_finalize(nope_encoder_t* e) {
  NOPE_CHECK(e, "null encoder");
  return e->finalize();
}

int nope_encoder_encode(nope_encoder_t* e, const float* images, int B, float* out, void* stream) {
  NOPE_CHECK(e && e->finalized, "encoder not finalized");
  NOPE_CHECK(images && out, "null images / out pointer");
  NOPE_CHECK(B >= 1, "B must be >= 1");
  NOPE_CUDA(cudaSetDevice(e->device));
  constexpr int kChunk = 32;
// ... 538 lines not shown
```

### nope_b200/csrc/wgmma.cuh

```cuda
#pragma once
#include <stdint.h>

namespace nope {

__device__ __forceinline__ void wgmma_fence() { asm volatile("wgmma.fence.sync.aligned;" ::: "memory"); }
__device__ __forceinline__ void wgmma_commit() { asm volatile("wgmma.commit_group.sync.aligned;" ::: "memory"); }
template <int N>
__device__ __forceinline__ void wgmma_wait() { asm volatile("wgmma.wait_group.sync.aligned %0;" ::"n"(N) : "memory"); }

constexpr uint64_t kWgDescK = (static_cast<uint64_t>(1) << 16) | (static_cast<uint64_t>(1024 >> 4) << 32) |
                              (static_cast<uint64_t>(1) << 62);
__device__ __forceinline__ uint64_t wg_desc_k(const void* p) {
  return kWgDescK | static_cast<uint64_t>((static_cast<uint32_t>(__cvta_generic_to_shared(p)) & 0x3FFFF) >> 4);
}

template <int N, bool BF16, int TRANS = 0>
struct Wgmma;

template <>
struct Wgmma<32, false, 0> {
  static __device__ __forceinline__ void mma(float (&d)[16], uint64_t a, uint64_t b, uint32_t accumulate) {
    asm volatile(
        "{\n\t.reg .pred p;\n\t"
        "setp.ne.b32 p, %18, 0;\n\t"
        "wgmma.mma_async.sync.aligned.m64n32k16.f32.f16.f16 "
        "{" 
        "%0, %1, %2, %3, %4, %5, %6, %7, %8, %9, %10, %11, %12, %13, %14, %15"
        "}, %16, %17, p, 1, 1, 0, 0;\n\t}\n"
        : "+f"(d[0]), "+f"(d[1]), "+f"(d[2]), "+f"(d[3]), "+f"(d[4]), "+f"(d[5]), "+f"(d[6]), "+f"(d[7]),
          "+f"(d[8]), "+f"(d[9]), "+f"(d[10]), "+f"(d[11]), "+f"(d[12]), "+f"(d[13]), "+f"(d[14]), "+f"(d[15])
        : "l"(a), "l"(b), "r"(accumulate));
  }
};
template <>
struct Wgmma<32, true, 0> {
  static __device__ __forceinline__ void mma(float (&d)[16], uint64_t a, uint64_t b, uint32_t accumulate) {
    asm volatile(
        "{\n\t.reg .pred p;\n\t"
        "setp.ne.b32 p, %18, 0;\n\t"
        "wgmma.mma_async.sync.aligned.m64n32k16.f32.bf16.bf16 "
        "{" 
        "%0, %1, %2, %3, %4, %5, %6, %7, %8, %9, %10, %11, %12, %13, %14, %15"
        "}, %16, %17, p, 1, 1, 0, 0;\n\t}\n"
        : "+f"(d[0]), "+f"(d[1]), "+f"(d[2]), "+f"(d[3]), "+f"(d[4]), "+f"(d[5]), "+f"(d[6]), "+f"(d[7]),
          "+f"(d[8]), "+f"(d[9]), "+f"(d[10]), "+f"(d[11]), "+f"(d[12]), "+f"(d[13]), "+f"(d[14]), "+f"(d[15])
        : "l"(a), "l"(b), "r"(accumulate));
  }
};
template <>
struct Wgmma<64, false, 0> {
  static __device__ __forceinline__ void mma(float (&d)[32], uint64_t a, uint64_t b, uint32_t accumulate) {
    asm volatile(
        "{\n\t.reg .pred p;\n\t"
        "setp.ne.b32 p, %34, 0;\n\t"
        "wgmma.mma_async.sync.aligned.m64n64k16.f32.f16.f16 "
        "{" 
        "%0, %1, %2, %3, %4, %5, %6, %7, %8, %9, %10, %11, %12, %13, %14, %15, "
        "%16, %17, %18, %19, %20, %21, %22, %23, %24, %25, %26, %27, %28, %29, %30, %31"
        "}, %32, %33, p, 1, 1, 0, 0;\n\t}\n"
        : "+f"(d[0]), "+f"(d[1]), "+f"(d[2]), "+f"(d[3]), "+f"(d[4]), "+f"(d[5]), "+f"(d[6]), "+f"(d[7]),
          "+f"(d[8]), "+f"(d[9]), "+f"(d[10]), "+f"(d[11]), "+f"(d[12]), "+f"(d[13]), "+f"(d[14]), "+f"(d[15]),
          "+f"(d[16]), "+f"(d[17]), "+f"(d[18]), "+f"(d[19]), "+f"(d[20]), "+f"(d[21]), "+f"(d[22]), "+f"(d[23]),
          "+f"(d[24]), "+f"(d[25]), "+f"(d[26]), "+f"(d[27]), "+f"(d[28]), "+f"(d[29]), "+f"(d[30]), "+f"(d[31])
        : "l"(a), "l"(b), "r"(accumulate));
  }
};
template <>
struct Wgmma<64, true, 0> {
  static __device__ __forceinline__ void mma(float (&d)[32], uint64_t a, uint64_t b, uint32_t accumulate) {
    asm volatile(
        "{\n\t.reg .pred p;\n\t"
        "setp.ne.b32 p, %34, 0;\n\t"
        "wgmma.mma_async.sync.aligned.m64n64k16.f32.bf16.bf16 "
        "{" 
        "%0, %1, %2, %3, %4, %5, %6, %7, %8, %9, %10, %11, %12, %13, %14, %15, "
        "%16, %17, %18, %19, %20, %21, %22, %23, %24, %25, %26, %27, %28, %29, %30, %31"
        "}, %32, %33, p, 1, 1, 0, 0;\n\t}\n"
        : "+f"(d[0]), "+f"(d[1]), "+f"(d[2]), "+f"(d[3]), "+f"(d[4]), "+f"(d[5]), "+f"(d[6]), "+f"(d[7]),
          "+f"(d[8]), "+f"(d[9]), "+f"(d[10]), "+f"(d[11]), "+f"(d[12]), "+f"(d[13]), "+f"(d[14]), "+f"(d[15]),
          "+f"(d[16]), "+f"(d[17]), "+f"(d[18]), "+f"(d[19]), "+f"(d[20]), "+f"(d[21]), "+f"(d[22]), "+f"(d[23]),
          "+f"(d[24]), "+f"(d[25]), "+f"(d[26]), "+f"(d[27]), "+f"(d[28]), "+f"(d[29]), "+f"(d[30]), "+f"(d[31])
        : "l"(a), "l"(b), "r"(accumulate));
  }
};
template <>
struct Wgmma<96, false, 0> {
  static __device__ __forceinline__ void mma(float (&d)[48], uint64_t a, uint64_t b, uint32_t accumulate) {
    asm volatile(
        "{\n\t.reg .pred p;\n\t"
        "setp.ne.b32 p, %50, 0;\n\t"
        "wgmma.mma_async.sync.aligned.m64n96k16.f32.f16.f16 "
        "{" 
        "%0, %1, %2, %3, %4, %5, %6, %7, %8, %9, %10, %11, %12, %13, %14, %15, "
        "%16, %17, %18, %19, %20, %21, %22, %23, %24, %25, %26, %27, %28, %29, %30, %31, "
        "%32, %33, %34, %35, %36, %37, %38, %39, %40, %41, %42, %43, %44, %45, %46, %47"
        "}, %48, %49, p, 1, 1, 0, 0;\n\t}\n"
        : "+f"(d[0]), "+f"(d[1]), "+f"(d[2]), "+f"(d[3]), "+f"(d[4]), "+f"(d[5]), "+f"(d[6]), "+f"(d[7]),
          "+f"(d[8]), "+f"(d[9]), "+f"(d[10]), "+f"(d[11]), "+f"(d[12]), "+f"(d[13]), "+f"(d[14]), "+f"(d[15]),
          "+f"(d[16]), "+f"(d[17]), "+f"(d[18]), "+f"(d[19]), "+f"(d[20]), "+f"(d[21]), "+f"(d[22]), "+f"(d[23]),
          "+f"(d[24]), "+f"(d[25]), "+f"(d[26]), "+f"(d[27]), "+f"(d[28]), "+f"(d[29]), "+f"(d[30]), "+f"(d[31]),
          "+f"(d[32]), "+f"(d[33]), "+f"(d[34]), "+f"(d[35]), "+f"(d[36]), "+f"(d[37]), "+f"(d[38]), "+f"(d[39]),
          "+f"(d[40]), "+f"(d[41]), "+f"(d[42]), "+f"(d[43]), "+f"(d[44]), "+f"(d[45]), "+f"(d[46]), "+f"(d[47])
        : "l"(a), "l"(b), "r"(accumulate));
  }
};
template <>
struct Wgmma<96, true, 0> {
  static __device__ __forceinline__ void mma(float (&d)[48], uint64_t a, uint64_t b, uint32_t accumulate) {
    asm volatile(
        "{\n\t.reg .pred p;\n\t"
        "setp.ne.b32 p, %50, 0;\n\t"
        "wgmma.mma_async.sync.aligned.m64n96k16.f32.bf16.bf16 "
        "{" 
        "%0, %1, %2, %3, %4, %5, %6, %7, %8, %9, %10, %11, %12, %13, %14, %15, "
        "%16, %17, %18, %19, %20, %21, %22, %23, %24, %25, %26, %27, %28, %29, %30, %31, "
        "%32, %33, %34, %35, %36, %37, %38, %39, %40, %41, %42, %43, %44, %45, %46, %47"
        "}, %48, %49, p, 1, 1, 0, 0;\n\t}\n"
        : "+f"(d[0]), "+f"(d[1]), "+f"(d[2]), "+f"(d[3]), "+f"(d[4]), "+f"(d[5]), "+f"(d[6]), "+f"(d[7]),
          "+f"(d[8]), "+f"(d[9]), "+f"(d[10]), "+f"(d[11]), "+f"(d[12]), "+f"(d[13]), "+f"(d[14]), "+f"(d[15]),
          "+f"(d[16]), "+f"(d[17]), "+f"(d[18]), "+f"(d[19]), "+f"(d[20]), "+f"(d[21]), "+f"(d[22]), "+f"(d[23]),
          "+f"(d[24]), "+f"(d[25]), "+f"(d[26]), "+f"(d[27]), "+f"(d[28]), "+f"(d[29]), "+f"(d[30]), "+f"(d[31]),
          "+f"(d[32]), "+f"(d[33]), "+f"(d[34]), "+f"(d[35]), "+f"(d[36]), "+f"(d[37]), "+f"(d[38]), "+f"(d[39]),
          "+f"(d[40]), "+f"(d[41]), "+f"(d[42]), "+f"(d[43]), "+f"(d[44]), "+f"(d[45]), "+f"(d[46]), "+f"(d[47])
        : "l"(a), "l"(b), "r"(accumulate));
  }
};
template <>
struct Wgmma<128, false, 0> {
  static __device__ __forceinline__ void mma(float (&d)[64], uint64_t a, uint64_t b, uint32_t accumulate) {
    asm volatile(
        "{\n\t.reg .pred p;\n\t"
        "setp.ne.b32 p, %66, 0;\n\t"
        "wgmma.mma_async.sync.aligned.m64n128k16.f32.f16.f16 "
        "{" 
        "%0, %1, %2, %3, %4, %5, %6, %7, %8, %9, %10, %11, %12, %13, %14, %15, "
        "%16, %17, %18, %19, %20, %21, %22, %23, %24, %25, %26, %27, %28, %29, %30, %31, "
        "%32, %33, %34, %35, %36, %37, %38, %39, %40, %41, %42, %43, %44, %45, %46, %47, "
        "%48, %49, %50, %51, %52, %53, %54, %55, %56, %57, %58, %59, %60, %61, %62, %63"
        "}, %64, %65, p, 1, 1, 0, 0;\n\t}\n"
        : "+f"(d[0]), "+f"(d[1]), "+f"(d[2]), "+f"(d[3]), "+f"(d[4]), "+f"(d[5]), "+f"(d[6]), "+f"(d[7]),
          "+f"(d[8]), "+f"(d[9]), "+f"(d[10]), "+f"(d[11]), "+f"(d[12]), "+f"(d[13]), "+f"(d[14]), "+f"(d[15]),
          "+f"(d[16]), "+f"(d[17]), "+f"(d[18]), "+f"(d[19]), "+f"(d[20]), "+f"(d[21]), "+f"(d[22]), "+f"(d[23]),
          "+f"(d[24]), "+f"(d[25]), "+f"(d[26]), "+f"(d[27]), "+f"(d[28]), "+f"(d[29]), "+f"(d[30]), "+f"(d[31]),
          "+f"(d[32]), "+f"(d[33]), "+f"(d[34]), "+f"(d[35]), "+f"(d[36]), "+f"(d[37]), "+f"(d[38]), "+f"(d[39]),
          "+f"(d[40]), "+f"(d[41]), "+f"(d[42]), "+f"(d[43]), "+f"(d[44]), "+f"(d[45]), "+f"(d[46]), "+f"(d[47]),
          "+f"(d[48]), "+f"(d[49]), "+f"(d[50]), "+f"(d[51]), "+f"(d[52]), "+f"(d[53]), "+f"(d[54]), "+f"(d[55]),
          "+f"(d[56]), "+f"(d[57]), "+f"(d[58]), "+f"(d[59]), "+f"(d[60]), "+f"(d[61]), "+f"(d[62]), "+f"(d[63])
        : "l"(a), "l"(b), "r"(accumulate));
  }
};
template <>
struct Wgmma<128, false, 1> {
  static __device__ __forceinline__ void mma(float (&d)[64], uint64_t a, uint64_t b, uint32_t accumulate) {
    asm volatile(
        "{\n\t.reg .pred p;\n\t"
        "setp.ne.b32 p, %66, 0;\n\t"
        "wgmma.mma_async.sync.aligned.m64n128k16.f32.f16.f16 "
        "{" 
        "%0, %1, %2, %3, %4, %5, %6, %7, %8, %9, %10, %11, %12, %13, %14, %15, "
        "%16, %17, %18, %19, %20, %21, %22, %23, %24, %25, %26, %27, %28, %29, %30, %31, "
        "%32, %33, %34, %35, %36, %37, %38, %39, %40, %41, %42, %43, %44, %45, %46, %47, "
        "%48, %49, %50, %51, %52, %53, %54, %55, %56, %57, %58, %59, %60, %61, %62, %63"
        "}, %64, %65, p, 1, 1, 1, 1;\n\t}\n"
        : "+f"(d[0]), "+f"(d[1]), "+f"(d[2]), "+f"(d[3]), "+f"(d[4]), "+f"(d[5]), "+f"(d[6]), "+f"(d[7]),
          "+f"(d[8]), "+f"(d[9]), "+f"(d[10]), "+f"(d[11]), "+f"(d[12]), "+f"(d[13]), "+f"(d[14]), "+f"(d[15]),
          "+f"(d[16]), "+f"(d[17]), "+f"(d[18]), "+f"(d[19]), "+f"(d[20]), "+f"(d[21]), "+f"(d[22]), "+f"(d[23]),
          "+f"(d[24]), "+f"(d[25]), "+f"(d[26]), "+f"(d[27]), "+f"(d[28]), "+f"(d[29]), "+f"(d[30]), "+f"(d[31]),
          "+f"(d[32]), "+f"(d[33]), "+f"(d[34]), "+f"(d[35]), "+f"(d[36]), "+f"(d[37]), "+f"(d[38]), "+f"(d[39]),
          "+f"(d[40]), "+f"(d[41]), "+f"(d[42]), "+f"(d[43]), "+f"(d[44]), "+f"(d[45]), "+f"(d[46]), "+f"(d[47]),
          "+f"(d[48]), "+f"(d[49]), "+f"(d[50]), "+f"(d[51]), "+f"(d[52]), "+f"(d[53]), "+f"(d[54]), "+f"(d[55]),
          "+f"(d[56]), "+f"(d[57]), "+f"(d[58]), "+f"(d[59]), "+f"(d[60]), "+f"(d[61]), "+f"(d[62]), "+f"(d[63])
        : "l"(a), "l"(b), "r"(accumulate));
  }
};
template <>
struct Wgmma<128, true, 0> {
  static __device__ __forceinline__ void mma(float (&d)[64], uint64_t a, uint64_t b, uint32_t accumulate) {
    asm volatile(
        "{\n\t.reg .pred p;\n\t"
        "setp.ne.b32 p, %66, 0;\n\t"
        "wgmma.mma_async.sync.aligned.m64n128k16.f32.bf16.bf16 "
        "{" 
        "%0, %1, %2, %3, %4, %5, %6, %7, %8, %9, %10, %11, %12, %13, %14, %15, "
        "%16, %17, %18, %19, %20, %21, %22, %23, %24, %25, %26, %27, %28, %29, %30, %31, "
        "%32, %33, %34, %35, %36, %37, %38, %39, %40, %41, %42, %43, %44, %45, %46, %47, "
        "%48, %49, %50, %51, %52, %53, %54, %55, %56, %57, %58, %59, %60, %61, %62, %63"
        "}, %64, %65, p, 1, 1, 0, 0;\n\t}\n"
        : "+f"(d[0]), "+f"(d[1]), "+f"(d[2]), "+f"(d[3]), "+f"(d[4]), "+f"(d[5]), "+f"(d[6]), "+f"(d[7]),
          "+f"(d[8]), "+f"(d[9]), "+f"(d[10]), "+f"(d[11]), "+f"(d[12]), "+f"(d[13]), "+f"(d[14]), "+f"(d[15]),
          "+f"(d[16]), "+f"(d[17]), "+f"(d[18]), "+f"(d[19]), "+f"(d[20]), "+f"(d[21]), "+f"(d[22]), "+f"(d[23]),
          "+f"(d[24]), "+f"(d[25]), "+f"(d[26]), "+f"(d[27]), "+f"(d[28]), "+f"(d[29]), "+f"(d[30]), "+f"(d[31]),
          "+f"(d[32]), "+f"(d[33]), "+f"(d[34]), "+f"(d[35]), "+f"(d[36]), "+f"(d[37]), "+f"(d[38]), "+f"(d[39]),
          "+f"(d[40]), "+f"(d[41]), "+f"(d[42]), "+f"(d[43]), "+f"(d[44]), "+f"(d[45]), "+f"(d[46]), "+f"(d[47]),
          "+f"(d[48]), "+f"(d[49]), "+f"(d[50]), "+f"(d[51]), "+f"(d[52]), "+f"(d[53]), "+f"(d[54]), "+f"(d[55]),
          "+f"(d[56]), "+f"(d[57]), "+f"(d[58]), "+f"(d[59]), "+f"(d[60]), "+f"(d[61]), "+f"(d[62]), "+f"(d[63])
        : "l"(a), "l"(b), "r"(accumulate));
  }
};
template <>
struct Wgmma<128, true, 1> {
  static __device__ __forceinline__ void mma(float (&d)[64], uint64_t a, uint64_t b, uint32_t accumulate) {
    asm volatile(
        "{\n\t.reg .pred p;\n\t"
        "setp.ne.b32 p, %66, 0;\n\t"
        "wgmma.mma_async.sync.aligned.m64n128k16.f32.bf16.bf16 "
        "{" 
        "%0, %1, %2, %3, %4, %5, %6, %7, %8, %9, %10, %11, %12, %13, %14, %15, "
        "%16, %17, %18, %19, %20, %21, %22, %23, %24, %25, %26, %27, %28, %29, %30, %31, "
        "%32, %33, %34, %35, %36, %37, %38, %39, %40, %41, %42, %43, %44, %45, %46, %47, "
        "%48, %49, %50, %51, %52, %53, %54, %55, %56, %57, %58, %59, %60, %61, %62, %63"
        "}, %64, %65, p, 1, 1, 1, 1;\n\t}\n"
        : "+f"(d[0]), "+f"(d[1]), "+f"(d[2]), "+f"(d[3]), "+f"(d[4]), "+f"(d[5]), "+f"(d[6]), "+f"(d[7]),
          "+f"(d[8]), "+f"(d[9]), "+f"(d[10]), "+f"(d[11]), "+f"(d[12]), "+f"(d[13]), "+f"(d[14]), "+f"(d[15]),
          "+f"(d[16]), "+f"(d[17]), "+f"(d[18]), "+f"(d[19]), "+f"(d[20]), "+f"(d[21]), "+f"(d[22]), "+f"(d[23]),
          "+f"(d[24]), "+f"(d[25]), "+f"(d[26]), "+f"(d[27]), "+f"(d[28]), "+f"(d[29]), "+f"(d[30]), "+f"(d[31]),
          "+f"(d[32]), "+f"(d[33]), "+f"(d[34]), "+f"(d[35]), "+f"(d[36]), "+f"(d[37]), "+f"(d[38]), "+f"(d[39]),
          "+f"(d[40]), "+f"(d[41]), "+f"(d[42]), "+f"(d[43]), "+f"(d[44]), "+f"(d[45]), "+f"(d[46]), "+f"(d[47]),
          "+f"(d[48]), "+f"(d[49]), "+f"(d[50]), "+f"(d[51]), "+f"(d[52]), "+f"(d[53]), "+f"(d[54]), "+f"(d[55]),
          "+f"(d[56]), "+f"(d[57]), "+f"(d[58]), "+f"(d[59]), "+f"(d[60]), "+f"(d[61]), "+f"(d[62]), "+f"(d[63])
        : "l"(a), "l"(b), "r"(accumulate));
  }
};

template <int N>
__device__ __forceinline__ void wg_store_acc(float* tile, int ld, int c0, const float (&d0)[N / 2], const float (&d1)[N / 2]) {
  const int t = threadIdx.x & 127, wq = t >> 5, l = t & 31;
  const int r = 16 * wq + (l >> 2), c = c0 + 2 * (l & 3);
#pragma unroll
  for (int i = 0; i < N / 8; ++i) {
    *reinterpret_cast<float2*>(tile + (size_t)r * ld + c + 8 * i) = make_float2(d0[4 * i], d0[4 * i + 1]);
    *reinterpret_cast<float2*>(tile + (size_t)(r + 8) * ld + c + 8 * i) = make_float2(d0[4 * i + 2], d0[4 * i + 3]);
    *reinterpret_cast<float2*>(tile + (size_t)(r + 64) * ld + c + 8 * i) = make_float2(d1[4 * i], d1[4 * i + 1]);
    *reinterpret_cast<float2*>(tile + (size_t)(r + 72) * ld + c + 8 * i) = make_float2(d1[4 * i + 2], d1[4 * i + 3]);
  }
}

__device__ __forceinline__ void acc_ld_32(const float* src, uint32_t (&v)[32]) {
#pragma unroll
  for (int j = 0; j < 8; ++j) {
    const float4 f = *reinterpret_cast<const float4*>(src + 4 * j);
    v[4 * j] = __float_as_uint(f.x);
    v[4 * j + 1] = __float_as_uint(f.y);
    v[4 * j + 2] = __float_as_uint(f.z);
    v[4 * j + 3] = __float_as_uint(f.w);
  }
}

}
```

Before: 12380.

## Split conv mainloop by M rows with full-width WGMMA and setmaxnreg register split

Changes the conv mainloop partitioning so that each math warpgroup owns 64 rows of the M tile and issues a full-BN-wide wgmma (up to n256), instead of splitting columns across warpgroups. With 2+ warpgroups each does one m64 slice; with one it does two. When a third warpgroup is present it skips the mainloop and only joins the barriers. Adds setmaxnreg-based register reallocation from the control warps to the math warps so the larger accumulators fit, and sets empty-barrier arrival counts to match the MMA warps. Per-launch shape columns are also added to the profiling dump. The risks are higher register pressure and a changed barrier count, which may cause spills or an imbalance across warpgroups.

```diff
diff --git a/nope_b200/csrc/conv_tc.cuh b/nope_b200/csrc/conv_tc.cuh
--- a/nope_b200/csrc/conv_tc.cuh
+++ b/nope_b200/csrc/conv_tc.cuh
@@ -111,23 +111,25 @@
 
 __host__ __device__ constexpr int acc_ld(int BN) { return BN + 4; }
 
-template <int NS, int STAGES, int kStageBytes, int kABytes, bool BF>
+__host__ __device__ constexpr int conv_mma_warps(int NW) { return NW < 2 ? 4 * NW : 8; }
+
+template <int N, int NH, int STAGES, int kStageBytes, int kABytes, bool BF>
 __device__ __forceinline__ void conv_mma_loop(const ConvParams& p, const uint8_t* smem, uint64_t* full_bar,
-                                              uint64_t* empty_bar, int& stage, uint32_t& phase, int wg,
-                                              float (&d0)[NS / 2], float (&d1)[NS / 2]) {
+                                              uint64_t* empty_bar, int& stage, uint32_t& phase, int a_blk,
+                                              float (&d)[NH][N / 2]) {
   const int lane = threadIdx.x & 31;
   int prev = -1;
   for (int ks = 0; ks < p.ksteps; ++ks) {
     mbar_wait(&full_bar[stage], phase);
     const uint8_t* sa = smem + stage * kStageBytes;
-    const uint64_t adesc = wg_desc_k(sa);
-    const uint64_t bdesc = wg_desc_k(sa + kABytes + wg * NS * 128);
+    const uint64_t adesc = wg_desc_k(sa + a_blk * (64 * 128));
+    const uint64_t bdesc = wg_desc_k(sa + kABytes);
     wgmma_fence();
 #pragma unroll
     for (int k = 0; k < kBK / 16; ++k) {
       const uint32_t acc = (ks | k) != 0 ? 1u : 0u;
-      Wgmma<NS, BF>::mma(d0, adesc + 2 * k, bdesc + 2 * k, acc);
-      Wgmma<NS, BF>::mma(d1, adesc + 512 + 2 * k, bdesc + 2 * k, acc);
+#pragma unroll
+      for (int h = 0; h < NH; ++h) Wgmma<N, BF>::mma(d[h], adesc + 512 * h + 2 * k, bdesc + 2 * k, acc);
     }
     wgmma_commit();
     wgmma_wait<1>();
@@ -139,20 +141,28 @@
   if (prev >= 0 && lane == 0) mbar_arrive(&empty_bar[prev]);
 }
 
-template <int BN, int NW, int STAGES, int kStageBytes, int kABytes>
+template <int BN, int NW, int STAGES, int kStageBytes, int kABytes, bool MMA = true>
 __device__ __forceinline__ void conv_mma_tile(const ConvParams& p, uint8_t* smem, uint64_t* full_bar,
                                               uint64_t* empty_bar, int& stage, uint32_t& phase, float* s_acc) {
-  constexpr int NS = BN / NW;
-  static_assert(NS % 32 == 0 && NS <= 128, "columns per warpgroup");
+  static_assert(NW >= 1 && NW <= 3 && BN % 64 == 0 && BN <= 256, "mainloop warpgroups / tile width");
+  constexpr int NH = NW >= 2 ? 1 : 2;
   const int wg = (threadIdx.x >> 7) - 1;
-  float d0[NS / 2], d1[NS / 2];
-#pragma unroll
-  for (int i = 0; i < NS / 2; ++i) { d0[i] = 0.f; d1[i] = 0.f; }
-  if (p.bf16) conv_mma_loop<NS, STAGES, kStageBytes, kABytes, true>(p, smem, full_bar, empty_bar, stage, phase, wg, d0, d1);
-  else conv_mma_loop<NS, STAGES, kStageBytes, kABytes, false>(p, smem, full_bar, empty_bar, stage, phase, wg, d0, d1);
-  asm volatile("bar.sync 2, %0;" ::"n"(NW * 128) : "memory");
-  wg_store_acc<NS>(s_acc, acc_ld(BN), wg * NS, d0, d1);
-  asm volatile("bar.sync 2, %0;" ::"n"(NW * 128) : "memory");
+  static_assert(MMA || NW == 3, "only the third of three warpgroups skips the mainloop");
+  if constexpr (MMA) {
+    float d[NH][BN / 2];
+#pragma unroll
+    for (int h = 0; h < NH; ++h)
+#pragma unroll
+      for (int i = 0; i < BN / 2; ++i) d[h][i] = 0.f;
+    if (p.bf16) conv_mma_loop<BN, NH, STAGES, kStageBytes, kABytes, true>(p, smem, full_bar, empty_bar, stage, phase, wg, d);
+    else conv_mma_loop<BN, NH, STAGES, kStageBytes, kABytes, false>(p, smem, full_bar, empty_bar, stage, phase, wg, d);
+    asm volatile("barrier.sync 2, %0;" ::"n"(NW * 128) : "memory");
+#pragma unroll
+    for (int h = 0; h < NH; ++h) wg_store_acc64<BN>(s_acc, acc_ld(BN), 64 * (wg + h), d[h]);
+  } else {
+    asm volatile("barrier.sync 2, %0;" ::"n"(NW * 128) : "memory");
+  }
+  asm volatile("barrier.sync 2, %0;" ::"n"(NW * 128) : "memory");
 }
 
 __device__ __forceinline__ void acc_release(uint64_t* tempty, int lane) {
@@ -387,7 +397,7 @@
   if (warp == 1 && lane == 0) {
     for (int s = 0; s < STAGES; ++s) {
       mbar_init(&full_bar[s], 1);
-      mbar_init(&empty_bar[s], kEpiWarps);
+      mbar_init(&empty_bar[s], conv_mma_warps(2));
     }
     mbar_init(tempty_bar, kEpiWarps);
     fence_mbar_init();
diff --git a/nope_b200/csrc/conv_tc2.cuh b/nope_b200/csrc/conv_tc2.cuh
--- a/nope_b200/csrc/conv_tc2.cuh
+++ b/nope_b200/csrc/conv_tc2.cuh
@@ -101,7 +101,7 @@
 __host__ __device__ constexpr int gn_epi_warps(int BN) { return 4 * (BN / 64); }
 __host__ __device__ constexpr int gn_threads(int BN) { return 128 + 32 * gn_epi_warps(BN); }
 
-template <int BN, int STAGES>
+template <int BN, int STAGES, bool MMA>
 __device__ __forceinline__ void conv_gn_epilogue_loop(const ConvParams& p, uint8_t* smem, uint64_t* full_bar,
                                                       uint64_t* empty_bar, uint64_t* tempty_bar, uint64_t* res_bar,
                                                       int tile0, int tile_step, int num_tiles, uint32_t rank) {
@@ -204,7 +204,7 @@
     NOPE_EPI_BAR();
     NOPE_TS(1);
     if (!(g.dbg & 16)) fetch_pb(tile + tile_step);
-    conv_mma_tile<BN, BN / 64, STAGES, S::kStageBytes, S::kABytes>(p, smem, full_bar, empty_bar, kstage, kphase, s_acc);
+    conv_mma_tile<BN, BN / 64, STAGES, S::kStageBytes, S::kABytes, MMA>(p, smem, full_bar, empty_bar, kstage, kphase, s_acc);
     NOPE_TS(2);
 
     uint32_t a[64];
@@ -596,7 +596,7 @@
 }
 
 
-template <int BN, int STAGES>
+template <int BN, int STAGES, bool MMA>
 __device__ __forceinline__ void conv_gn2_math_warps(const ConvParams& p, uint8_t* smem, uint8_t* gsm,
                                                     const Gn2Bars& B, int tile0, int tile_step, int num_tiles,
                                                     uint32_t rank) {
@@ -657,7 +657,7 @@
     const __half* pb_row = g.pb + (size_t)(img_ok ? img0 + it : 0) * g.pb_stride + g.pb_off + n_chan0 + cc * 64;
     if (g.pb && live) asm volatile("prefetch.global.L1 [%0];" ::"l"(pb_row));
 
-    conv_mma_tile<BN, BN / 64, STAGES, S::kStageBytes, S::kABytes>(p, smem, B.full, B.empty, kstage, kphase, s_acc);
+    conv_mma_tile<BN, BN / 64, STAGES, S::kStageBytes, S::kABytes, MMA>(p, smem, B.full, B.empty, kstage, kphase, s_acc);
     NOPE_TS(1);
     uint32_t a[64];
     {
@@ -1203,12 +1203,25 @@
   if (lane == 0) tma_store_wait_all();
 }
 
+__host__ __device__ constexpr int conv2_threads(int BN, int EPI) { return EPI >= 3 ? gn_threads(BN) : kConvThreads; }
+__host__ __device__ constexpr int conv2_ctl_regs(int EPI) { return EPI == 4 ? 80 : 56; }
+__host__ __device__ constexpr int conv2_launch_regs(int threads) { return 65536 / threads / 8 * 8; }
+__host__ __device__ constexpr int conv2_math_regs(int threads, int EPI) {
+  return (conv2_launch_regs(threads) * (threads / 128) - conv2_ctl_regs(EPI)) / (threads / 128 - 1) / 8 * 8;
+}
+
 template <int BN, int STAGES, int EPI>
-__global__ void __cluster_dims__(2, 1, 1) __launch_bounds__(EPI >= 3 ? gn_threads(BN) : kConvThreads, 1)
+__global__ void __cluster_dims__(2, 1, 1) __launch_bounds__(conv2_threads(BN, EPI), 1)
 conv_tc2_kernel(const __grid_constant__ ConvParams p) {
   using S = Conv2Smem<BN, STAGES, EPI>;
   static_assert(BN % 64 == 0 && BN <= 256, "BN must be a multiple of 64");
-  constexpr int kMathWarps = EPI >= 3 ? gn_epi_warps(BN) : kEpiWarps;
+  constexpr int kThreads = conv2_threads(BN, EPI);
+  constexpr int kMathWarps = kThreads / 32 - 4;
+  constexpr bool kRegSplit = kThreads > 256;
+  constexpr int kCtlRegs = conv2_ctl_regs(EPI);
+  constexpr int kMathRegs = conv2_math_regs(kThreads, EPI);
+  static_assert(!kRegSplit || (kMathRegs <= 256 && kCtlRegs + (kThreads / 128 - 1) * kMathRegs <=
+                               conv2_launch_regs(kThreads) * (kThreads / 128)), "register split");
 
   extern __shared__ uint8_t smem_raw[];
   uint8_t* smem = reinterpret_cast<uint8_t*>((reinterpret_cast<uintptr_t>(smem_raw) + 1023) &
@@ -1238,7 +1251,7 @@
   if (warp == 1 && lane == 0) {
     for (int s = 0; s < STAGES; ++s) {
       mbar_init(&full_bar[s], 1);
-      mbar_init(&empty_bar[s], kMathWarps);
+      mbar_init(&empty_bar[s], conv_mma_warps(kMathWarps / 4));
     }
     mbar_init(tempty_bar, kMathWarps);
     mbar_init(res_bar, 1);
@@ -1256,8 +1269,17 @@
   }
   __syncthreads();
   pdl_sync();
-
-  if (warp == 0) {
+  auto gn2_bars = [&] {
+    Gn2Bars B;
+    B.full = full_bar; B.empty = empty_bar; B.tempty = tempty_bar; B.res[0] = res_bar; B.res[1] = &gn2_bar[7];
+    B.part = &gn2_bar[0]; B.stats = &gn2_bar[1]; B.tabfree = &gn2_bar[3]; B.out = &gn2_bar[5];
+    return B;
+  };
+  uint8_t* gsm = smem + S::kGnOffset;
+
+  if (warp < 4) {
+    if constexpr (kRegSplit) setmaxnreg_dec<kCtlRegs>();
+    if (warp == 0) {
     int stage = 0;
     uint32_t phase = 0;
     int iter = 0;
@@ -1305,21 +1327,31 @@
         }
       }
     }
-  } else if (EPI == 4 && warp >= 2) {
-    if constexpr (EPI == 4) {
-      Gn2Bars B;
-      B.full = full_bar; B.empty = empty_bar; B.tempty = tempty_bar; B.res[0] = res_bar; B.res[1] = &gn2_bar[7];
-      B.part = &gn2_bar[0]; B.stats = &gn2_bar[1]; B.tabfree = &gn2_bar[3]; B.out = &gn2_bar[5];
-      uint8_t* gsm = smem + S::kGnOffset;
+    } else if constexpr (EPI == 4) {
+      const Gn2Bars B = gn2_bars();
       if (warp == 2) conv_gn2_store_warp<BN, STAGES>(p, smem, gsm, B, tile0, tile_step, num_tiles, rank);
       else if (warp == 3) conv_gn2_stats_warp<BN, STAGES>(p, gsm, B, tile0, tile_step, num_tiles, rank);
-      else conv_gn2_math_warps<BN, STAGES>(p, smem, gsm, B, tile0, tile_step, num_tiles, rank);
-    }
-  } else if (warp >= 4 && EPI == 3) {
-    if constexpr (EPI == 3)
-      conv_gn_epilogue_loop<BN, STAGES>(p, smem, full_bar, empty_bar, tempty_bar, res_bar, tile0, tile_step,
-                                        num_tiles, rank);
-  } else if (warp >= 4) {
+    }
+  } else if constexpr (EPI == 4) {
+    if constexpr (kRegSplit) setmaxnreg_inc<kMathRegs>();
+    if (warp >= 12) {
+      if constexpr (kMathWarps == 12) conv_gn2_math_warps<BN, STAGES, false>(p, smem, gsm, gn2_bars(), tile0, tile_step, num_tiles, rank);
+    } else {
+      conv_gn2_math_warps<BN, STAGES, true>(p, smem, gsm, gn2_bars(), tile0, tile_step, num_tiles, rank);
+    }
+  } else if constexpr (EPI == 3) {
+    if constexpr (kRegSplit) setmaxnreg_inc<kMathRegs>();
+    if (warp >= 12) {
+      if constexpr (kMathWarps == 12)
+        conv_gn_epilogue_loop<BN, STAGES, false>(p, smem, full_bar, empty_bar, tempty_bar, res_bar, tile0, tile_step,
+                                                 num_tiles, rank);
+    } else {
+      conv_gn_epilogue_loop<BN, STAGES, true>(p, smem, full_bar, empty_bar, tempty_bar, res_bar, tile0, tile_step,
+                                              num_tiles, rank);
+    }
+  } else {
+    static_assert(kRegSplit, "the plain epilogues run 384 threads");
+    setmaxnreg_inc<kMathRegs>();
     const int e = warp - 4;
     const int etid = threadIdx.x - 128;
     int kstage = 0;
@@ -1401,7 +1433,7 @@
       cudaLaunchConfig_t cfg;
       memset(&cfg, 0, sizeof cfg);
       cfg.gridDim = dim3(num_sms, 1, 1);
-      cfg.blockDim = dim3(EPI >= 3 ? gn_threads(BN) : kConvThreads, 1, 1);
+      cfg.blockDim = dim3(conv2_threads(BN, EPI), 1, 1);
       cfg.dynamicSmemBytes = S::kTotal;
       cudaLaunchAttribute at;
       at.id = cudaLaunchAttributeClusterDimension;
@@ -1421,7 +1453,7 @@
   cudaLaunchConfig_t cfg;
   memset(&cfg, 0, sizeof cfg);
   cfg.gridDim = dim3(2 * clusters, 1, 1);
-  cfg.blockDim = dim3(EPI >= 3 ? gn_threads(BN) : kConvThreads, 1, 1);
+  cfg.blockDim = dim3(conv2_threads(BN, EPI), 1, 1);
   cfg.dynamicSmemBytes = S::kTotal;
   cfg.stream = stream;
   cudaLaunchAttribute at;
diff --git a/nope_b200/csrc/nope_b200.cu b/nope_b200/csrc/nope_b200.cu
--- a/nope_b200/csrc/nope_b200.cu
+++ b/nope_b200/csrc/nope_b200.cu
@@ -756,9 +756,11 @@
     prof_ev.push_back(e1);
     prof_flops.push_back(2.0 * (double)n_img * So * So * (double)L.cout * (double)ksteps * 64.0);
     prof_alg.push_back(2.0 * (double)n_img * So * So * (double)L.cout * (double)L.K);
+    prof_shape.push_back(make_int4(So, L.mode, L.cout, L.K));
     return rc;
   }
   std::vector<double> prof_alg;
+  std::vector<int4> prof_shape;
 
   static int gn_nslab(int hw, int n_img) {
     int ns = 1;
@@ -1197,6 +1199,7 @@
   u->prof_ev.clear();
   u->prof_flops.clear();
   u->prof_alg.clear();
+  u->prof_shape.clear();
   u->profile = enable != 0;
   return 0;
 }
@@ -1216,11 +1219,13 @@
   }
   if (const char* path = std::getenv("NOPE_PROF_DUMP")) {
     if (FILE* f = std::fopen(path, "a")) {
-      std::fprintf(f, "# launch,ms,executed_gflop,algorithmic_gflop\n");
+      std::fprintf(f, "# launch,ms,executed_gflop,algorithmic_gflop,res,mode,cout,k\n");
       for (size_t i = 0; i < u->prof_flops.size(); ++i) {
         float t = 0.f;
         cudaEventElapsedTime(&t, u->prof_ev[2 * i], u->prof_ev[2 * i + 1]);
-        std::fprintf(f, "%zu,%.4f,%.3f,%.3f\n", i, t, u->prof_flops[i] / 1e9, u->prof_alg[i] / 1e9);
+        const int4 sh = u->prof_shape[i];
+        std::fprintf(f, "%zu,%.4f,%.3f,%.3f,%d,%d,%d,%d\n", i, t, u->prof_flops[i] / 1e9, u->prof_alg[i] / 1e9, sh.x,
+                     sh.y, sh.z, sh.w);
       }
       std::fclose(f);
     }
diff --git a/nope_b200/csrc/wgmma.cuh b/nope_b200/csrc/wgmma.cuh
--- a/nope_b200/csrc/wgmma.cuh
+++ b/nope_b200/csrc/wgmma.cuh
@@ -7,6 +7,10 @@
 __device__ __forceinline__ void wgmma_commit() { asm volatile("wgmma.commit_group.sync.aligned;" ::: "memory"); }
 template <int N>
 __device__ __forceinline__ void wgmma_wait() { asm volatile("wgmma.wait_group.sync.aligned %0;" ::"n"(N) : "memory"); }
+template <int R>
+__device__ __forceinline__ void setmaxnreg_dec() { asm volatile("setmaxnreg.dec.sync.aligned.u32 %0;" ::"n"(R)); }
+template <int R>
+__device__ __forceinline__ void setmaxnreg_inc() { asm volatile("setmaxnreg.inc.sync.aligned.u32 %0;" ::"n"(R)); }
 
 constexpr uint64_t kWgDescK = (static_cast<uint64_t>(1) << 16) | (static_cast<uint64_t>(1024 >> 4) << 32) |
                               (static_cast<uint64_t>(1) << 62);
@@ -84,48 +88,6 @@
   }
 };
 template <>
-struct Wgmma<96, false, 0> {
-  static __device__ __forceinline__ void mma(float (&d)[48], uint64_t a, uint64_t b, uint32_t accumulate) {
-    asm volatile(
-        "{\n\t.reg .pred p;\n\t"
-        "setp.ne.b32 p, %50, 0;\n\t"
-        "wgmma.mma_async.sync.aligned.m64n96k16.f32.f16.f16 "
-        "{" 
-        "%0, %1, %2, %3, %4, %5, %6, %7, %8, %9, %10, %11, %12, %13, %14, %15, "
-        "%16, %17, %18, %19, %20, %21, %22, %23, %24, %25, %26, %27, %28, %29, %30, %31, "
-        "%32, %33, %34, %35, %36, %37, %38, %39, %40, %41, %42, %43, %44, %45, %46, %47"
-        "}, %48, %49, p, 1, 1, 0, 0;\n\t}\n"
-        : "+f"(d[0]), "+f"(d[1]), "+f"(d[2]), "+f"(d[3]), "+f"(d[4]), "+f"(d[5]), "+f"(d[6]), "+f"(d[7]),
-          "+f"(d[8]), "+f"(d[9]), "+f"(d[10]), "+f"(d[11]), "+f"(d[12]), "+f"(d[13]), "+f"(d[14]), "+f"(d[15]),
-          "+f"(d[16]), "+f"(d[17]), "+f"(d[18]), "+f"(d[19]), "+f"(d[20]), "+f"(d[21]), "+f"(d[22]), "+f"(d[23]),
-          "+f"(d[24]), "+f"(d[25]), "+f"(d[26]), "+f"(d[27]), "+f"(d[28]), "+f"(d[29]), "+f"(d[30]), "+f"(d[31]),
-          "+f"(d[32]), "+f"(d[33]), "+f"(d[34]), "+f"(d[35]), "+f"(d[36]), "+f"(d[37]), "+f"(d[38]), "+f"(d[39]),
-          "+f"(d[40]), "+f"(d[41]), "+f"(d[42]), "+f"(d[43]), "+f"(d[44]), "+f"(d[45]), "+f"(d[46]), "+f"(d[47])
-        : "l"(a), "l"(b), "r"(accumulate));
-  }
-};
-template <>
-struct Wgmma<96, true, 0> {
-  static __device__ __forceinline__ void mma(float (&d)[48], uint64_t a, uint64_t b, uint32_t accumulate) {
-    asm volatile(
-        "{\n\t.reg .pred p;\n\t"
-        "setp.ne.b32 p, %50, 0;\n\t"
-        "wgmma.mma_async.sync.aligned.m64n96k16.f32.bf16.bf16 "
-        "{" 
-        "%0, %1, %2, %3, %4, %5, %6, %7, %8, %9, %10, %11, %12, %13, %14, %15, "
-        "%16, %17, %18, %19, %20, %21, %22, %23, %24, %25, %26, %27, %28, %29, %30, %31, "
-        "%32, %33, %34, %35, %36, %37, %38, %39, %40, %41, %42, %43, %44, %45, %46, %47"
-        "}, %48, %49, p, 1, 1, 0, 0;\n\t}\n"
-        : "+f"(d[0]), "+f"(d[1]), "+f"(d[2]), "+f"(d[3]), "+f"(d[4]), "+f"(d[5]), "+f"(d[6]), "+f"(d[7]),
-          "+f"(d[8]), "+f"(d[9]), "+f"(d[10]), "+f"(d[11]), "+f"(d[12]), "+f"(d[13]), "+f"(d[14]), "+f"(d[15]),
-          "+f"(d[16]), "+f"(d[17]), "+f"(d[18]), "+f"(d[19]), "+f"(d[20]), "+f"(d[21]), "+f"(d[22]), "+f"(d[23]),
-          "+f"(d[24]), "+f"(d[25]), "+f"(d[26]), "+f"(d[27]), "+f"(d[28]), "+f"(d[29]), "+f"(d[30]), "+f"(d[31]),
-          "+f"(d[32]), "+f"(d[33]), "+f"(d[34]), "+f"(d[35]), "+f"(d[36]), "+f"(d[37]), "+f"(d[38]), "+f"(d[39]),
-          "+f"(d[40]), "+f"(d[41]), "+f"(d[42]), "+f"(d[43]), "+f"(d[44]), "+f"(d[45]), "+f"(d[46]), "+f"(d[47])
-        : "l"(a), "l"(b), "r"(accumulate));
-  }
-};
-template <>
 struct Wgmma<128, false, 0> {
   static __device__ __forceinline__ void mma(float (&d)[64], uint64_t a, uint64_t b, uint32_t accumulate) {
     asm volatile(
@@ -218,6 +180,139 @@
           "+f"(d[40]), "+f"(d[41]), "+f"(d[42]), "+f"(d[43]), "+f"(d[44]), "+f"(d[45]), "+f"(d[46]), "+f"(d[47]),
           "+f"(d[48]), "+f"(d[49]), "+f"(d[50]), "+f"(d[51]), "+f"(d[52]), "+f"(d[53]), "+f"(d[54]), "+f"(d[55]),
           "+f"(d[56]), "+f"(d[57]), "+f"(d[58]), "+f"(d[59]), "+f"(d[60]), "+f"(d[61]), "+f"(d[62]), "+f"(d[63])
+        : "l"(a), "l"(b), "r"(accumulate));
+  }
+};
+
+template <>
+struct Wgmma<192, false, 0> {
+  static __device__ __forceinline__ void mma(float (&d)[96], uint64_t a, uint64_t b, uint32_t accumulate) {
+    asm volatile(
+        "{\n\t.reg .pred p;\n\t"
+        "setp.ne.b32 p, %98, 0;\n\t"
+        "wgmma.mma_async.sync.aligned.m64n192k16.f32.f16.f16 "
+        "{" 
+        "%0, %1, %2, %3, %4, %5, %6, %7, %8, %9, %10, %11, %12, %13, %14, %15, "
+        "%16, %17, %18, %19, %20, %21, %22, %23, %24, %25, %26, %27, %28, %29, %30, %31, "
+        "%32, %33, %34, %35, %36, %37, %38, %39, %40, %41, %42, %43, %44, %45, %46, %47, "
+        "%48, %49, %50, %51, %52, %53, %54, %55, %56, %57, %58, %59, %60, %61, %62, %63, "
+        "%64, %65, %66, %67, %68, %69, %70, %71, %72, %73, %74, %75, %76, %77, %78, %79, "
+        "%80, %81, %82, %83, %84, %85, %86, %87, %88, %89, %90, %91, %92, %93, %94, %95"
+        "}, %96, %97, p, 1, 1, 0, 0;\n\t}\n"
+        : "+f"(d[0]), "+f"(d[1]), "+f"(d[2]), "+f"(d[3]), "+f"(d[4]), "+f"(d[5]), "+f"(d[6]), "+f"(d[7]),
+          "+f"(d[8]), "+f"(d[9]), "+f"(d[10]), "+f"(d[11]), "+f"(d[12]), "+f"(d[13]), "+f"(d[14]), "+f"(d[15]),
+          "+f"(d[16]), "+f"(d[17]), "+f"(d[18]), "+f"(d[19]), "+f"(d[20]), "+f"(d[21]), "+f"(d[22]), "+f"(d[23]),
+          "+f"(d[24]), "+f"(d[25]), "+f"(d[26]), "+f"(d[27]), "+f"(d[28]), "+f"(d[29]), "+f"(d[30]), "+f"(d[31]),
+          "+f"(d[32]), "+f"(d[33]), "+f"(d[34]), "+f"(d[35]), "+f"(d[36]), "+f"(d[37]), "+f"(d[38]), "+f"(d[39]),
+          "+f"(d[40]), "+f"(d[41]), "+f"(d[42]), "+f"(d[43]), "+f"(d[44]), "+f"(d[45]), "+f"(d[46]), "+f"(d[47]),
+          "+f"(d[48]), "+f"(d[49]), "+f"(d[50]), "+f"(d[51]), "+f"(d[52]), "+f"(d[53]), "+f"(d[54]), "+f"(d[55]),
+          "+f"(d[56]), "+f"(d[57]), "+f"(d[58]), "+f"(d[59]), "+f"(d[60]), "+f"(d[61]), "+f"(d[62]), "+f"(d[63]),
+          "+f"(d[64]), "+f"(d[65]), "+f"(d[66]), "+f"(d[67]), "+f"(d[68]), "+f"(d[69]), "+f"(d[70]), "+f"(d[71]),
+          "+f"(d[72]), "+f"(d[73]), "+f"(d[74]), "+f"(d[75]), "+f"(d[76]), "+f"(d[77]), "+f"(d[78]), "+f"(d[79]),
+          "+f"(d[80]), "+f"(d[81]), "+f"(d[82]), "+f"(d[83]), "+f"(d[84]), "+f"(d[85]), "+f"(d[86]), "+f"(d[87]),
+          "+f"(d[88]), "+f"(d[89]), "+f"(d[90]), "+f"(d[91]), "+f"(d[92]), "+f"(d[93]), "+f"(d[94]), "+f"(d[95])
+        : "l"(a), "l"(b), "r"(accumulate));
+  }
+};
+template <>
+struct Wgmma<192, true, 0> {
+  static __device__ __forceinline__ void mma(float (&d)[96], uint64_t a, uint64_t b, uint32_t accumulate) {
+    asm volatile(
+        "{\n\t.reg .pred p;\n\t"
+        "setp.ne.b32 p, %98, 0;\n\t"
+        "wgmma.mma_async.sync.aligned.m64n192k16.f32.bf16.bf16 "
+        "{" 
+        "%0, %1, %2, %3, %4, %5, %6, %7, %8, %9, %10, %11, %12, %13, %14, %15, "
+        "%16, %17, %18, %19, %20, %21, %22, %23, %24, %25, %26, %27, %28, %29, %30, %31, "
+        "%32, %33, %34, %35, %36, %37, %38, %39, %40, %41, %42, %43, %44, %45, %46, %47, "
+        "%48, %49, %50, %51, %52, %53, %54, %55, %56, %57, %58, %59, %60, %61, %62, %63, "
+        "%64, %65, %66, %67, %68, %69, %70, %71, %72, %73, %74, %75, %76, %77, %78, %79, "
+        "%80, %81, %82, %83, %84, %85, %86, %87, %88, %89, %90, %91, %92, %93, %94, %95"
+        "}, %96, %97, p, 1, 1, 0, 0;\n\t}\n"
+        : "+f"(d[0]), "+f"(d[1]), "+f"(d[2]), "+f"(d[3]), "+f"(d[4]), "+f"(d[5]), "+f"(d[6]), "+f"(d[7]),
+          "+f"(d[8]), "+f"(d[9]), "+f"(d[10]), "+f"(d[11]), "+f"(d[12]), "+f"(d[13]), "+f"(d[14]), "+f"(d[15]),
+          "+f"(d[16]), "+f"(d[17]), "+f"(d[18]), "+f"(d[19]), "+f"(d[20]), "+f"(d[21]), "+f"(d[22]), "+f"(d[23]),
+          "+f"(d[24]), "+f"(d[25]), "+f"(d[26]), "+f"(d[27]), "+f"(d[28]), "+f"(d[29]), "+f"(d[30]), "+f"(d[31]),
+          "+f"(d[32]), "+f"(d[33]), "+f"(d[34]), "+f"(d[35]), "+f"(d[36]), "+f"(d[37]), "+f"(d[38]), "+f"(d[39]),
+          "+f"(d[40]), "+f"(d[41]), "+f"(d[42]), "+f"(d[43]), "+f"(d[44]), "+f"(d[45]), "+f"(d[46]), "+f"(d[47]),
+          "+f"(d[48]), "+f"(d[49]), "+f"(d[50]), "+f"(d[51]), "+f"(d[52]), "+f"(d[53]), "+f"(d[54]), "+f"(d[55]),
+          "+f"(d[56]), "+f"(d[57]), "+f"(d[58]), "+f"(d[59]), "+f"(d[60]), "+f"(d[61]), "+f"(d[62]), "+f"(d[63]),
+          "+f"(d[64]), "+f"(d[65]), "+f"(d[66]), "+f"(d[67]), "+f"(d[68]), "+f"(d[69]), "+f"(d[70]), "+f"(d[71]),
+          "+f"(d[72]), "+f"(d[73]), "+f"(d[74]), "+f"(d[75]), "+f"(d[76]), "+f"(d[77]), "+f"(d[78]), "+f"(d[79]),
+          "+f"(d[80]), "+f"(d[81]), "+f"(d[82]), "+f"(d[83]), "+f"(d[84]), "+f"(d[85]), "+f"(d[86]), "+f"(d[87]),
+          "+f"(d[88]), "+f"(d[89]), "+f"(d[90]), "+f"(d[91]), "+f"(d[92]), "+f"(d[93]), "+f"(d[94]), "+f"(d[95])
+        : "l"(a), "l"(b), "r"(accumulate));
+  }
+};
+template <>
+struct Wgmma<256, false, 0> {
+  static __device__ __forceinline__ void mma(float (&d)[128], uint64_t a, uint64_t b, uint32_t accumulate) {
+    asm volatile(
+        "{\n\t.reg .pred p;\n\t"
+        "setp.ne.b32 p, %130, 0;\n\t"
+        "wgmma.mma_async.sync.aligned.m64n256k16.f32.f16.f16 "
+        "{" 
+        "%0, %1, %2, %3, %4, %5, %6, %7, %8, %9, %10, %11, %12, %13, %14, %15, "
+        "%16, %17, %18, %19, %20, %21, %22, %23, %24, %25, %26, %27, %28, %29, %30, %31, "
+        "%32, %33, %34, %35, %36, %37, %38, %39, %40, %41, %42, %43, %44, %45, %46, %47, "
+        "%48, %49, %50, %51, %52, %53, %54, %55, %56, %57, %58, %59, %60, %61, %62, %63, "
+        "%64, %65, %66, %67, %68, %69, %70, %71, %72, %73, %74, %75, %76, %77, %78, %79, "
+        "%80, %81, %82, %83, %84, %85, %86, %87, %88, %89, %90, %91, %92, %93, %94, %95, "
+        "%96, %97, %98, %99, %100, %101, %102, %103, %104, %105, %106, %107, %108, %109, %110, %111, "
+        "%112, %113, %114, %115, %116, %117, %118, %119, %120, %121, %122, %123, %124, %125, %126, %127"
+        "}, %128, %129, p, 1, 1, 0, 0;\n\t}\n"
+        : "+f"(d[0]), "+f"(d[1]), "+f"(d[2]), "+f"(d[3]), "+f"(d[4]), "+f"(d[5]), "+f"(d[6]), "+f"(d[7]),
+          "+f"(d[8]), "+f"(d[9]), "+f"(d[10]), "+f"(d[11]), "+f"(d[12]), "+f"(d[13]), "+f"(d[14]), "+f"(d[15]),
+          "+f"(d[16]), "+f"(d[17]), "+f"(d[18]), "+f"(d[19]), "+f"(d[20]), "+f"(d[21]), "+f"(d[22]), "+f"(d[23]),
+          "+f"(d[24]), "+f"(d[25]), "+f"(d[26]), "+f"(d[27]), "+f"(d[28]), "+f"(d[29]), "+f"(d[30]), "+f"(d[31]),
+          "+f"(d[32]), "+f"(d[33]), "+f"(d[34]), "+f"(d[35]), "+f"(d[36]), "+f"(d[37]), "+f"(d[38]), "+f"(d[39]),
+          "+f"(d[40]), "+f"(d[41]), "+f"(d[42]), "+f"(d[43]), "+f"(d[44]), "+f"(d[45]), "+f"(d[46]), "+f"(d[47]),
+          "+f"(d[48]), "+f"(d[49]), "+f"(d[50]), "+f"(d[51]), "+f"(d[52]), "+f"(d[53]), "+f"(d[54]), "+f"(d[55]),
+          "+f"(d[56]), "+f"(d[57]), "+f"(d[58]), "+f"(d[59]), "+f"(d[60]), "+f"(d[61]), "+f"(d[62]), "+f"(d[63]),
+          "+f"(d[64]), "+f"(d[65]), "+f"(d[66]), "+f"(d[67]), "+f"(d[68]), "+f"(d[69]), "+f"(d[70]), "+f"(d[71]),
+          "+f"(d[72]), "+f"(d[73]), "+f"(d[74]), "+f"(d[75]), "+f"(d[76]), "+f"(d[77]), "+f"(d[78]), "+f"(d[79]),
+          "+f"(d[80]), "+f"(d[81]), "+f"(d[82]), "+f"(d[83]), "+f"(d[84]), "+f"(d[85]), "+f"(d[86]), "+f"(d[87]),
+          "+f"(d[88]), "+f"(d[89]), "+f"(d[90]), "+f"(d[91]), "+f"(d[92]), "+f"(d[93]), "+f"(d[94]), "+f"(d[95]),
+          "+f"(d[96]), "+f"(d[97]), "+f"(d[98]), "+f"(d[99]), "+f"(d[100]), "+f"(d[101]), "+f"(d[102]), "+f"(d[103]),
+          "+f"(d[104]), "+f"(d[105]), "+f"(d[106]), "+f"(d[107]), "+f"(d[108]), "+f"(d[109]), "+f"(d[110]), "+f"(d[111]),
+          "+f"(d[112]), "+f"(d[113]), "+f"(d[114]), "+f"(d[115]), "+f"(d[116]), "+f"(d[117]), "+f"(d[118]), "+f"(d[119]),
+          "+f"(d[120]), "+f"(d[121]), "+f"(d[122]), "+f"(d[123]), "+f"(d[124]), "+f"(d[125]), "+f"(d[126]), "+f"(d[127])
+        : "l"(a), "l"(b), "r"(accumulate));
+  }
+};
+template <>
+struct Wgmma<256, true, 0> {
+  static __device__ __forceinline__ void mma(float (&d)[128], uint64_t a, uint64_t b, uint32_t accumulate) {
+    asm volatile(
+        "{\n\t.reg .pred p;\n\t"
+        "setp.ne.b32 p, %130, 0;\n\t"
+        "wgmma.mma_async.sync.aligned.m64n256k16.f32.bf16.bf16 "
+        "{" 
+        "%0, %1, %2, %3, %4, %5, %6, %7, %8, %9, %10, %11, %12, %13, %14, %15, "
+        "%16, %17, %18, %19, %20, %21, %22, %23, %24, %25, %26, %27, %28, %29, %30, %31, "
+        "%32, %33, %34, %35, %36, %37, %38, %39, %40, %41, %42, %43, %44, %45, %46, %47, "
+        "%48, %49, %50, %51, %52, %53, %54, %55, %56, %57, %58, %59, %60, %61, %62, %63, "
+        "%64, %65, %66, %67, %68, %69, %70, %71, %72, %73, %74, %75, %76, %77, %78, %79, "
+        "%80, %81, %82, %83, %84, %85, %86, %87, %88, %89, %90, %91, %92, %93, %94, %95, "
+        "%96, %97, %98, %99, %100, %101, %102, %103, %104, %105, %106, %107, %108, %109, %110, %111, "
+        "%112, %113, %114, %115, %116, %117, %118, %119, %120, %121, %122, %123, %124, %125, %126, %127"
+        "}, %128, %129, p, 1, 1, 0, 0;\n\t}\n"
+        : "+f"(d[0]), "+f"(d[1]), "+f"(d[2]), "+f"(d[3]), "+f"(d[4]), "+f"(d[5]), "+f"(d[6]), "+f"(d[7]),
+          "+f"(d[8]), "+f"(d[9]), "+f"(d[10]), "+f"(d[11]), "+f"(d[12]), "+f"(d[13]), "+f"(d[14]), "+f"(d[15]),
+          "+f"(d[16]), "+f"(d[17]), "+f"(d[18]), "+f"(d[19]), "+f"(d[20]), "+f"(d[21]), "+f"(d[22]), "+f"(d[23]),
+          "+f"(d[24]), "+f"(d[25]), "+f"(d[26]), "+f"(d[27]), "+f"(d[28]), "+f"(d[29]), "+f"(d[30]), "+f"(d[31]),
+          "+f"(d[32]), "+f"(d[33]), "+f"(d[34]), "+f"(d[35]), "+f"(d[36]), "+f"(d[37]), "+f"(d[38]), "+f"(d[39]),
+          "+f"(d[40]), "+f"(d[41]), "+f"(d[42]), "+f"(d[43]), "+f"(d[44]), "+f"(d[45]), "+f"(d[46]), "+f"(d[47]),
+          "+f"(d[48]), "+f"(d[49]), "+f"(d[50]), "+f"(d[51]), "+f"(d[52]), "+f"(d[53]), "+f"(d[54]), "+f"(d[55]),
+          "+f"(d[56]), "+f"(d[57]), "+f"(d[58]), "+f"(d[59]), "+f"(d[60]), "+f"(d[61]), "+f"(d[62]), "+f"(d[63]),
+          "+f"(d[64]), "+f"(d[65]), "+f"(d[66]), "+f"(d[67]), "+f"(d[68]), "+f"(d[69]), "+f"(d[70]), "+f"(d[71]),
+          "+f"(d[72]), "+f"(d[73]), "+f"(d[74]), "+f"(d[75]), "+f"(d[76]), "+f"(d[77]), "+f"(d[78]), "+f"(d[79]),
+          "+f"(d[80]), "+f"(d[81]), "+f"(d[82]), "+f"(d[83]), "+f"(d[84]), "+f"(d[85]), "+f"(d[86]), "+f"(d[87]),
+          "+f"(d[88]), "+f"(d[89]), "+f"(d[90]), "+f"(d[91]), "+f"(d[92]), "+f"(d[93]), "+f"(d[94]), "+f"(d[95]),
+          "+f"(d[96]), "+f"(d[97]), "+f"(d[98]), "+f"(d[99]), "+f"(d[100]), "+f"(d[101]), "+f"(d[102]), "+f"(d[103]),
+          "+f"(d[104]), "+f"(d[105]), "+f"(d[106]), "+f"(d[107]), "+f"(d[108]), "+f"(d[109]), "+f"(d[110]), "+f"(d[111]),
+          "+f"(d[112]), "+f"(d[113]), "+f"(d[114]), "+f"(d[115]), "+f"(d[116]), "+f"(d[117]), "+f"(d[118]), "+f"(d[119]),
+          "+f"(d[120]), "+f"(d[121]), "+f"(d[122]), "+f"(d[123]), "+f"(d[124]), "+f"(d[125]), "+f"(d[126]), "+f"(d[127])
         : "l"(a), "l"(b), "r"(accumulate));
   }
 };
@@ -235,6 +330,17 @@
   }
 }
 
+template <int N>
+__device__ __forceinline__ void wg_store_acc64(float* tile, int ld, int r0, const float (&d)[N / 2]) {
+  const int t = threadIdx.x & 127, wq = t >> 5, l = t & 31;
+  const int r = r0 + 16 * wq + (l >> 2), c = 2 * (l & 3);
+#pragma unroll
+  for (int i = 0; i < N / 8; ++i) {
+    *reinterpret_cast<float2*>(tile + (size_t)r * ld + c + 8 * i) = make_float2(d[4 * i], d[4 * i + 1]);
+    *reinterpret_cast<float2*>(tile + (size_t)(r + 8) * ld + c + 8 * i) = make_float2(d[4 * i + 2], d[4 * i + 3]);
+  }
+}
+
 __device__ __forceinline__ void acc_ld_32(const float* src, uint32_t (&v)[32]) {
 #pragma unroll
   for (int j = 0; j < 8; ++j) {
```

New measurement: 13630 (median of 6 runs). 1.1x the previous value.
